# aimi-lab/robust-pose-estimator

Measured on AMD Instinct MI355X. Metric: stereo-pair pose solves/sec (640x512, 8 solver iters), higher is better.
Workload: dtype f32 (RAFT / geometry) + f64 (SE(3) solve), as the reference; 1 GPU; PoseNet.infer, 640x512 stereo frame pairs, 16 per GPU per step (RAFT batch 32), 12 GRU iters, lbfgs x8 SE(3) solve, weight heads on; frames_per_gpu=16, height=512, width=640, raft_iters=12, solver=lbfgs, solver_iters=8, parallelism=frames sharded x1

## Files before the change

include/rpe.h:

```cpp
#ifndef RPE_H
#define RPE_H

#include <stddef.h>
#include <stdint.h>

#ifdef __cplusplus
extern "C" {
#endif

#define RPE_OK 0
#define RPE_E_BADARG (-1)
#define RPE_E_LAUNCH (-2)
#define RPE_E_UNSUPPORTED (-3)

#define RPE_F32 0
#define RPE_F64 1
#define RPE_F16 2
#define RPE_F32X3 3

#define RPE_SOLVER_LBFGS 0
#define RPE_SOLVER_GN 1

#define RPE_STOP_OPT_AT_START 1
#define RPE_STOP_GTD 2
// ... 48 lines not shown
    int reserved;
} rpe_solve_opts;
#define RPE_SOLVE_LAUNCH_PER_EVALUATION 1
int rpe_pose_solve_ex(const float *flow, const float *pcl1, const float *pcl2, const float *w1, const float *w2,
                      const uint8_t *mask1, const uint8_t *mask2, const float *K, const float *loss_weight,
                      int n, int h, int w, int mode, int iters, const rpe_solve_opts *opts, double *T_out, float *vec7,
                      float *log6, int32_t *info, void *workspace, void *stream);

size_t rpe_pose_quality_workspace_bytes(int n, int h, int w);
int rpe_pose_quality(const float *flow, const float *pcl1, const float *pcl2, const float *w1, const float *w2,
                     const uint8_t *mask1, const uint8_t *mask2, const float *K, const float *loss_weight,
                     const double *T, int n, int h, int w, double *out, void *workspace, void *stream);

size_t rpe_pose_backward_workspace_bytes(int n, int h, int w);
int rpe_pose_backward_moments(const float *flow, const float *pcl1, const float *pcl2, const float *w1, const float *w2,
                              const uint8_t *mask1, const uint8_t *mask2, const float *K, const float *loss_weight,
                              const double *T, int n, int h, int w, double *out, void *workspace, void *stream);
int rpe_pose_backward_grads(const float *flow, const float *pcl1, const float *pcl2, const float *w1, const float *w2,
                            const uint8_t *mask1, const uint8_t *mask2, const float *K, const float *loss_weight,
                            const double *T, const double *u, int n, int h, int w, float *grad_flow, float *grad_pcl1,
                            float *grad_pcl2, float *grad_w1, float *grad_w2, void *stream);

int rpe_depth_backproject_warp(const float *stereo_flow2, const float *time_flow, const float *baseline,
                               const float *K, const float *depth1, const float *image1l, const float *image2l,
                               const float *stereo_flow1, const uint8_t *mask2, int n, int h, int w,
                               float *depth2, uint8_t *mask2_valid, float *pcl1, float *pcl2w, uint8_t *mask2w,
                               float *inp1, float *inp2, float *pcl2, void *stream);

int rpe_flow2depth(const float *stereo_flow, const float *baseline, int n, int h, int w, float *depth,
                   uint8_t *valid, void *stream);

int rpe_warp_taps(const float *flow, int n, int h, int w, int32_t *x0, int32_t *y0, int32_t *xn, int32_t *yn,
                  void *stream);

size_t rpe_depth_backproject_warp_backward_workspace_bytes(int n, int h, int w);
int rpe_depth_backproject_warp_backward(const float *stereo_flow2, const float *time_flow, const float *baseline,
                                        const float *K, const float *depth1, const float *image2l,
                                        const float *stereo_flow1, const uint8_t *mask2, int n, int h, int w,
                                        const float *grad_pcl1, const float *grad_pcl2w, const float *grad_inp1,
                                        const float *grad_inp2, float *grad_time_flow, float *grad_stereo_flow2,
                                        float *grad_stereo_flow1, float *grad_depth1, void *workspace, void *stream);
int rpe_flow2depth_backward(const float *stereo_flow, const float *baseline, const float *grad_depth, int n, int h, int w,
                            float *grad_stereo_flow, void *stream);

int rpe_upsample_convex_backward(const float *grad_up, const float *flow, const float *mask, int b, int h8, int w8, float *d_flow,
                                 float *d_mask, void *stream);
size_t rpe_conv_bwd_weight_workspace_bytes(int b, int cin, int cout, int h, int w, int kh, int kw);
int rpe_conv_bwd_weight(const float *x, long long x_batch_stride, const float *dy, long long dy_batch_stride, int b, int cin, int cout,
                        int h, int w, int kh, int kw, float scale, float *d_weight, float *d_bias, void *workspace, void *stream);
int rpe_conv3x3_to2_bwd_data(const float *dy, long long dy_batch_stride, const float *weight, const float *act,
                             long long act_batch_stride, int b, int c, int h, int w, float *dx, long long dx_batch_stride, void *stream);
int rpe_relu_backward(const float *grad, long long grad_batch_stride, const float *act, long long act_batch_stride, int b, int c, int hw,
                      float *out, long long out_batch_stride, void *stream);
int rpe_sum_groups(const float *parts, int groups, int b, int c, int hw, const float *bias, int relu, float *out, long long out_batch_stride,
                   void *stream);

int rpe_gru_gates_zr_recompute(const float *zr_pre, long long zr_batch_stride, const float *h, long long h_batch_stride, int b, int c, int hw,
                               float *z, long long z_batch_stride, float *r, long long r_batch_stride, float *rh, long long rh_batch_stride,
                               void *stream);
int rpe_gru_gates_h_recompute(const float *q_pre, long long qp_batch_stride, const float *z, long long z_batch_stride, const float *h,
                              long long h_batch_stride, int b, int c, int hw, float *q, long long q_batch_stride, float *h_new,
                              long long hn_batch_stride, void *stream);
int rpe_gru_gates_zq_backward(const float *d_h_new, long long d_batch_stride, const float *h, long long h_batch_stride, const float *z,
                              long long z_batch_stride, const float *q, long long q_batch_stride, int b, int c, int hw, float *d_z_pre,
                              long long dz_batch_stride, float *d_q_pre, long long dq_batch_stride, float *d_h, long long dh_batch_stride,
                              void *stream);
int rpe_gru_gates_r_backward(const float *d_rh, long long drh_batch_stride, const float *h, long long h_batch_stride, const float *r,
                             long long r_batch_stride, const float *d_h_in, long long dhi_batch_stride, int b, int c, int hw, float *d_r_pre,
                             long long dr_batch_stride, float *d_h_out, long long dho_batch_stride, void *stream);

size_t rpe_corr_grad_volume_floats(int b, int h8, int w8, int levels);
int rpe_corr_lookup_backward(const float *coords, const float *d_corr, int b, int h8, int w8, int levels, int radius, float *grad_volume,
                             void *stream);
size_t rpe_corr_build_backward_workspace_bytes(int b, int c, int h8, int w8, int levels);
int rpe_corr_build_backward(const float *grad_volume, const float *fmap1, const float *fmap2, int b, int c, int h8, int w8, int levels,
                            float *d_fmap1, float *d_fmap2, float *d_f2cat, void *workspace, void *stream);

size_t rpe_corr_pyramid_bytes(int b, int h8, int w8, int levels);
size_t rpe_corr_pyramid_bytes_ex(int b, int h8, int w8, int levels, int feature_dtype);
int rpe_corr_build(const float *fmap1, const float *fmap2, int b, int c, int h8, int w8, int levels,
                   void *pyramid, void *stream);
int rpe_corr_build_ex(const float *fmap1, const float *fmap2, int b, int c, int h8, int w8, int levels, int feature_dtype,
                      void *pyramid, void *stream);
int rpe_corr_lookup(const void *pyramid, const float *coords, int b, int h8, int w8, int levels, int radius,
                    float *out, void *stream);
int rpe_corr_lookup_ex(const void *pyramid, const float *coords, int b, int h8, int w8, int levels, int radius, int map_h, int map_w,
                       float *out, void *stream);
size_t rpe_corr_lookup_conv1x1_packed_floats(int cout, int cin);
int rpe_corr_lookup_conv1x1_pack(const float *weight, int cout, int cin, float *packed, void *stream);
int rpe_corr_lookup_conv1x1(const void *pyramid, const float *coords, int b, int h8, int w8, int levels, int radius, const float *packed,
                            const float *bias, int relu, float *out, long long out_batch_stride, float *out2, long long out2_batch_stride,
                            void *stream);
int rpe_corr_lookup_taps(const float *coords, int b, int h8, int w8, int levels, int32_t *x0, int32_t *y0,
                         void *stream);
int rpe_corr_lookup_rounds(const float *coords, int b, int h8, int w8, int levels, int32_t *rounds, int32_t *lines,
                           void *stream);
int rpe_corr_export_level(const void *pyramid, int b, int h8, int w8, int levels, int level, float *dense,
                          void *stream);

#define RPE_CORR_ALT_PAD 512
size_t rpe_corr_alt_bytes(int b, int c, int h8, int w8, int levels);
int rpe_corr_alt_prepare(const float *fmap1, const float *fmap2, int b, int c, int h8, int w8, int levels, void *scratch, void *stream);
int rpe_corr_alt_lookup(const void *scratch, const float *coords, int b, int c, int h8, int w8, int levels, int radius, float *out,
                        void *stream);
int rpe_corr_alt_lookup_ex(const void *scratch, const float *coords, int b, int c, int h8, int w8, int levels, int radius, int map_h, int map_w,
                           float *out, void *stream);
size_t rpe_corr_alt_bytes_ex(int b, int c, int h8, int w8, int levels, int feature_dtype);
int rpe_corr_alt_prepare_ex(const float *fmap1, const float *fmap2, int b, int c, int h8, int w8, int levels, int feature_dtype, void *scratch,
                            void *stream);
int rpe_corr_alt_lookup_dt(const void *scratch, const float *coords, int b, int c, int h8, int w8, int levels, int radius, int map_h, int map_w,
                           int feature_dtype, float *out, void *stream);

int rpe_gru_gates_zr(const float *zr_pre, const float *zr_bias, const float *zr_add, const float *h, int h_channels,
                     int b, int c, int hw, float *z_out, float *rh_out, int rh_channels, void *stream);
int rpe_gru_gates_h(const float *z, const float *q_pre, const float *q_bias, const float *q_add, const float *h,
                    int h_channels, int b, int c, int hw, float *h_out, int hout_channels, void *stream);
int rpe_bias_act(const float *x, const float *bias, int b, int c, int hw, int relu, float *out1, int out1_channels,
                 int out1_offset, float *out2, int out2_channels, int out2_offset, void *stream);
int rpe_instnorm_act(const float *x, const float *bias, int b, int c, int hw, float eps, int relu,
                     const float *residual, float *out, void *stream);
int rpe_affine_act(const float *x, const float *scale, const float *shift, int b, int c, int hw, int relu,
                   const float *residual, float *out, void *stream);
int rpe_copy_planes(const float *src, long long src_batch_stride, float *dst, long long dst_batch_stride, int b, int c, int hw,
                    void *stream);
int rpe_conv3x3_to2(const float *x, const float *weight, const float *bias, int b, int c, int h, int w,
                    const float *add, float *out, void *stream);
int rpe_conv3x3_to2_flow(const float *x, const float *weight, const float *bias, int b, int c, int h, int w,
                         const float *coords, float *coords_out, float *flow_out, float *dst1, long long dst1_batch_stride,
                         float *dst2, long long dst2_batch_stride, void *stream);
int rpe_flow_forward_interpolate(const float *flow, int b, int h, int w, float *out, void *stream);
int rpe_flow_seed(const float *flow_init, int b, int h, int w, float *coords_out, float *flow_out, float *dst1, long long dst1_batch_stride,
                  float *dst2, long long dst2_batch_stride, void *stream);
int rpe_upsample_convex(const float *flow, const float *mask, int b, int h8, int w8, float *out, void *stream);
int rpe_upsample_convex_ex(const float *flow, const float *mask, int b, int h8, int w8, int map_h, int map_w, float *out, void *stream);
int rpe_conv3x3_to2_flow_v(const float *x, const float *weight, const float *bias, int b, int c, int h, int w,
                           const float *coords, float *coords_out, float *flow_out, float *dst1, long long dst1_batch_stride,
                           float *dst2, long long dst2_batch_stride, int h_valid, int w_valid, void *stream);
int rpe_copy_rect(const float *src, long long src_batch_stride, long long src_plane_stride, int src_pitch, float *dst,
                  long long dst_batch_stride, long long dst_plane_stride, int dst_pitch, int b, int c, int h, int w, void *stream);

#define RPE_CONV_LINEAR 0
#define RPE_CONV_RELU 1
#define RPE_CONV_GATE_ZR 2
#define RPE_CONV_GATE_H 3
#define RPE_CONV_TANH 4
typedef struct rpe_conv_desc {
    const float *x;      long long x_batch_stride;
    const float *packed;
    const float *bias;
    const float *add;    long long add_batch_stride;
    float *out;          long long out_batch_stride;
    float *out2;         long long out2_batch_stride;
    const float *hidden; long long hidden_batch_stride;
    const float *zgate;  long long zgate_batch_stride;
    const float *scale;
    const float *residual; long long residual_batch_stride;
    float *stats;
    const float *pre_norm;
    int b, cin, cout, h, w, kh, kw, mode, gate_channels;
    int stride;
    int stats_tiles;
} rpe_conv_desc;
typedef struct rpe_conv_desc_v { rpe_conv_desc d; int h_valid, w_valid; } rpe_conv_desc_v;
int rpe_conv_wino_v(const rpe_conv_desc_v *desc, void *stream);
int rpe_conv_wino24_v(const rpe_conv_desc_v *desc, void *stream);
int rpe_conv_wino1d_v(const rpe_conv_desc_v *desc, void *stream);
int rpe_conv1x1_v(const rpe_conv_desc_v *desc, void *stream);
int rpe_enc_conv_wino_v(const rpe_conv_desc_v *desc, void *stream);
int rpe_enc_conv_wino24_v(const rpe_conv_desc_v *desc, void *stream);
int rpe_enc_conv_s2_v(const rpe_conv_desc_v *desc, void *stream);
int rpe_enc_conv_s2_m96_v(const rpe_conv_desc_v *desc, void *stream);
size_t rpe_conv_packed_floats(int cout, int cin, int kh, int kw);
int rpe_conv_pack(const float *weight, int cout, int cin, int kh, int kw, float *packed, void *stream);
int rpe_conv_fused(const rpe_conv_desc *desc, void *stream);
int rpe_conv_fused_m96(const rpe_conv_desc *desc, void *stream);
size_t rpe_conv_wino_packed_floats(int cout, int cin);
int rpe_conv_wino_stats_tiles(int h, int w);
int rpe_conv_wino_pack(const float *weight, int cout, int cin, float *packed, void *stream);
int rpe_conv_wino(const rpe_conv_desc *desc, void *stream);
size_t rpe_conv_wino24_packed_floats(int cout, int cin);
int rpe_conv_wino24_pack(const float *weight, int cout, int cin, float *packed, void *stream);
int rpe_conv_wino24(const rpe_conv_desc *desc, void *stream);
size_t rpe_conv_wino_x3_packed_bytes(int cout, int cin);
int rpe_conv_wino_x3_pack(const float *weight, int cout, int cin, void *packed, void *stream);
int rpe_conv_wino_x3(const rpe_conv_desc *desc, void *stream);
size_t rpe_conv_wino1d_packed_floats(int cout, int cin);
int rpe_conv_wino1d_pack(const float *weight, int cout, int cin, float *packed, void *stream);
int rpe_conv_wino1d(const rpe_conv_desc *desc, void *stream);
size_t rpe_conv_wino1d_x3_packed_bytes(int cout, int cin);
int rpe_conv_wino1d_x3_pack(const float *weight, int cout, int cin, void *packed, void *stream);
int rpe_conv_wino1d_x3(const rpe_conv_desc *desc, void *stream);
size_t rpe_conv1x1_packed_floats(int cout, int cin);
int rpe_conv1x1_pack(const float *weight, int cout, int cin, float *packed, void *stream);
int rpe_conv1x1(const rpe_conv_desc *desc, void *stream);
size_t rpe_conv1x1_x3_packed_bytes(int cout, int cin);
int rpe_conv1x1_x3_pack(const float *weight, int cout, int cin, void *packed, void *stream);
int rpe_conv1x1_x3(const rpe_conv_desc *desc, void *stream);
size_t rpe_conv_f16_packed_bytes(int cout, int cin, int kh, int kw);
int rpe_conv_f16_pack(const float *weight, int cout, int cin, int kh, int kw, void *packed, void *stream);
int rpe_conv_f16(const rpe_conv_desc *desc, void *stream);
int rpe_conv_direct(const float *x, long long x_batch_stride, const float *weight, const float *bias, int b, int cin, int cout,
                    int h, int w, int kh, int kw, int stride, int pad_h, int pad_w, int relu, float *out,
                    long long out_batch_stride, void *stream);
int rpe_conv_stats_tiles(int cout, int h, int w, int stride);
int rpe_conv_stats_tiles_batch(int cout, int h, int w, int stride, int b);
int rpe_instnorm_apply(const float *x, const float *partials, int tiles, int b, int c, int hw, float eps, int relu,
                       const float *residual, float *out, void *stream);
int rpe_instnorm_apply_ex(const float *x, const float *partials, int tiles, int b, int c, int hw, float eps, int relu,
                          const float *residual, const float *residual_mean_inv, float *out, void *stream);
int rpe_instnorm_finalize(const float *partials, int tiles, int b, int c, int hw, float eps, float *mean_inv, void *stream);
int rpe_instnorm_apply_v(const float *x, const float *mean_inv, int b, int c, int h, int w, int h_valid, int w_valid, int relu,
                         const float *residual, const float *residual_mean_inv, float *out, void *stream);

#define RPE_OP_CONV_FUSED 1
#define RPE_OP_CONV_WINO 2
#define RPE_OP_CONV_WINO1D 3
#define RPE_OP_CONV1X1 4
#define RPE_OP_CONV_WINO_X3 5
#define RPE_OP_CONV_WINO1D_X3 6
#define RPE_OP_CONV1X1_X3 7
#define RPE_OP_CORR_LOOKUP 8
#define RPE_OP_STEM_CONV 9
#define RPE_OP_FLOW_UPDATE 10
#define RPE_OP_COPY_PLANES 11
#define RPE_OP_INSTNORM_FINALIZE 12
#define RPE_OP_INSTNORM_APPLY 13
#define RPE_OP_UPSAMPLE_CONVEX 14
#define RPE_OP_CORR_BUILD 15
#define RPE_OP_LOOKUP_CONV1X1 16
#define RPE_OP_CONV_WINO24 17
#define RPE_OP_FLOW_SEED 18
#define RPE_OP_CONV_FUSED_M96 19
#define RPE_OP_CORR_ALT_PREPARE 20
#define RPE_OP_CORR_ALT_LOOKUP 21
#define RPE_OP_CONV_WINO_V 22
#define RPE_OP_CONV_WINO24_V 23
#define RPE_OP_CONV_WINO1D_V 24
#define RPE_OP_CONV1X1_V 25
#define RPE_OP_STEM_CONV_V 26
#define RPE_OP_FLOW_UPDATE_V 27
#define RPE_OP_CORR_LOOKUP_EX 28
#define RPE_OP_CORR_ALT_LOOKUP_EX 29
#define RPE_OP_UPSAMPLE_CONVEX_EX 30
#define RPE_OP_COPY_RECT 31
#define RPE_OP_EVENT_RECORD 32
#define RPE_OP_STREAM_WAIT 33
#define RPE_OP_ENC_CONV_WINO_V 34
#define RPE_OP_ENC_CONV_WINO24_V 35
#define RPE_OP_ENC_CONV_S2_V 36
#define RPE_OP_ENC_CONV_S2_M96_V 37
#define RPE_OP_INSTNORM_APPLY_V 38
#define RPE_OP_CORR_ALT_PREPARE_EX 39
#define RPE_OP_CORR_ALT_LOOKUP_DT 40
#define RPE_OP_CONV_F16 (RPE_OP_CORR_ALT_LOOKUP_DT + 1)
typedef struct rpe_op {
    int kind;
    int stream;
    const void *args;
} rpe_op;
typedef struct rpe_corr_lookup_args { const void *pyramid; const float *coords; int b, h8, w8, levels, radius; float *out; } rpe_corr_lookup_args;
typedef struct rpe_lookup_conv1x1_args {
    const void *pyramid; const float *coords; int b, h8, w8, levels, radius; const float *packed, *bias; int relu; float *out;
    long long out_batch_stride; float *out2; long long out2_batch_stride;
} rpe_lookup_conv1x1_args;
typedef struct rpe_corr_build_args { const float *fmap1, *fmap2; int b, c, h8, w8, levels, feature_dtype; void *pyramid; } rpe_corr_build_args;
typedef struct rpe_corr_alt_prepare_args { const float *fmap1, *fmap2; int b, c, h8, w8, levels; void *scratch; } rpe_corr_alt_prepare_args;
typedef struct rpe_corr_alt_lookup_args { const void *scratch; const float *coords; int b, c, h8, w8, levels, radius; float *out; } rpe_corr_alt_lookup_args;
typedef struct rpe_stem_conv_args {
    const float *image; int b, cin, h, w, stride; float div, mul, sub; const float *packed; int cout; const float *bias, *scale; int relu;
    float *out, *stats;
} rpe_stem_conv_args;
typedef struct rpe_flow_update_args {
    const float *x, *weight, *bias; int b, c, h, w; const float *coords; float *coords_out, *flow_out, *dst1; long long dst1_batch_stride;
    float *dst2; long long dst2_batch_stride;
} rpe_flow_update_args;
typedef struct rpe_flow_seed_args {
    const float *flow_init; int b, h, w; float *coords_out, *flow_out, *dst1; long long dst1_batch_stride; float *dst2; long long dst2_batch_stride;
} rpe_flow_seed_args;
typedef struct rpe_copy_planes_args { const float *src; long long src_batch_stride; float *dst; long long dst_batch_stride; int b, c, hw; } rpe_copy_planes_args;
typedef struct rpe_instnorm_finalize_args { const float *partials; int tiles, b, c, hw; float eps; float *mean_inv; } rpe_instnorm_finalize_args;
typedef struct rpe_instnorm_apply_args {
    const float *x, *partials; int tiles, b, c, hw; float eps; int relu; const float *residual, *residual_mean_inv; float *out;
} rpe_instnorm_apply_args;
typedef struct rpe_upsample_convex_args { const float *flow, *mask; int b, h8, w8; float *out; } rpe_upsample_convex_args;
typedef struct rpe_corr_lookup_ex_args { const void *pyramid; const float *coords; int b, h8, w8, levels, radius, map_h, map_w; float *out; } rpe_corr_lookup_ex_args;
typedef struct rpe_corr_alt_lookup_ex_args {
    const void *scratch; const float *coords; int b, c, h8, w8, levels, radius, map_h, map_w; float *out;
} rpe_corr_alt_lookup_ex_args;
typedef struct rpe_stem_conv_v_args {
    const float *image; int b, cin, h, w, stride; float div, mul, sub; const float *packed; int cout; const float *bias, *scale; int relu;
    float *out, *stats; int h_valid, w_valid;
} rpe_stem_conv_v_args;
typedef struct rpe_flow_update_v_args {
    const float *x, *weight, *bias; int b, c, h, w; const float *coords; float *coords_out, *flow_out, *dst1; long long dst1_batch_stride;
    float *dst2; long long dst2_batch_stride; int h_valid, w_valid;
} rpe_flow_update_v_args;
typedef struct rpe_upsample_convex_ex_args { const float *flow, *mask; int b, h8, w8, map_h, map_w; float *out; } rpe_upsample_convex_ex_args;
typedef struct rpe_copy_rect_args {
    const float *src; long long src_batch_stride, src_plane_stride; int src_pitch; float *dst; long long dst_batch_stride, dst_plane_stride;
    int dst_pitch, b, c, h, w;
} rpe_copy_rect_args;
typedef struct rpe_instnorm_apply_v_args {
    const float *x, *mean_inv; int b, c, h, w, h_valid, w_valid, relu; const float *residual, *residual_mean_inv; float *out;
} rpe_instnorm_apply_v_args;
typedef struct rpe_corr_alt_prepare_ex_args {
    const float *fmap1, *fmap2; int b, c, h8, w8, levels, feature_dtype; void *scratch;
} rpe_corr_alt_prepare_ex_args;
typedef struct rpe_corr_alt_lookup_dt_args {
    const void *scratch; const float *coords; int b, c, h8, w8, levels, radius, map_h, map_w, feature_dtype; float *out;
} rpe_corr_alt_lookup_dt_args;
int rpe_run_ops(const rpe_op *ops, int n_ops, void *const *streams, int n_streams, int *failed_op);

size_t rpe_unet_params_floats(int in_channels);
size_t rpe_unet_workspace_bytes(int b, int h8, int w8);
int rpe_unet_heads(const float *inp1, const float *inp2, const float *hidden, const float *context, long long hidden_batch_stride,
                   long long context_batch_stride, const float *params2d, const float *params3d, int b, int h8, int w8, int H, int W,
                   float *out2d, float *out3d, void *workspace, void *stream);

size_t rpe_unet_train_workspace_bytes(int n, int cin, int h8, int w8, int out_h, int out_w);
size_t rpe_unet_train_workspace_offset(int n, int cin, int h8, int w8, int index);
int rpe_unet_train_workspace_extent(int n, int cin, int h8, int w8, int index, int *extent);
size_t rpe_unet_train_grad_floats(int cin);
size_t rpe_unet_train_grad_offset(int cin, int index);
int rpe_unet_train_forward(const float *const *src, const int *src_channels, const long long *src_batch_strides, int nsrc,
                           const float *const *params, float *const *running_mean, float *const *running_var,
                           long long *const *num_batches_tracked, const float *momentum, const float *eps, int train_mask,
                           int n, int h8, int w8, int out_h, int out_w, int sigmoid, float *out, void *workspace, void *stream);
int rpe_unet_train_backward(const float *grad_out, const float *out, const float *const *src, const int *src_channels,
                            const long long *src_batch_strides, int nsrc, const float *const *params, int train_mask, int n, int h8, int w8,
                            int out_h, int out_w, int sigmoid, float *grad_params, float *grad_input, void *workspace, void *stream);

int rpe_stem_tiles(int h, int w, int stride);
size_t rpe_stem_packed_floats(int cout, int cin);
int rpe_stem_pack(const float *weight, int cout, int cin, float *packed, void *stream);
int rpe_stem_conv(const float *image, int b, int cin, int h, int w, int stride, float div, float mul, float sub,
                  const float *packed, int cout, const float *bias, const float *scale, int relu, float *out,
                  float *stats, void *stream);
int rpe_stem_conv_v(const float *image, int b, int cin, int h, int w, int stride, float div, float mul, float sub,
                    const float *packed, int cout, const float *bias, const float *scale, int relu, float *out,
                    float *stats, int h_valid, int w_valid, void *stream);

int rpe_mask_specularities(const uint8_t *img_hwc, const uint8_t *mask, int h, int w, int sum_threshold, uint8_t *out,
                           void *stream);
int rpe_resize_crop(const void *in, int in_is_u8_hwc, int c, int h, int w, int resized_h, int resized_w, int top, int left,
                    int out_h, int out_w, float *out, void *stream);
int rpe_resize_crop_mask(const uint8_t *in, int h, int w, int resized_h, int resized_w, int top, int left, int out_h,
                         int out_w, uint8_t *out, void *stream);
int rpe_remap_nearest(const void *src, int src_is_u8, int c, int h, int w, const float *mapx, const float *mapy, int out_h,
// ... 52 lines not shown
```

robust-pose-estimator_amd/_lib.py:

```python
import ctypes
import os
import subprocess

import torch

_HERE = os.path.dirname(os.path.abspath(__file__))
LIB_PATH = os.environ.get('RPE_HIP_LIBRARY', os.path.join(_HERE, 'librpe_hip.so'))
CSRC = os.path.join(_HERE, 'csrc')

_c = ctypes
_vp, _i, _i64, _d, _sz = _c.c_void_p, _c.c_int, _c.c_int64, _c.c_double, _c.c_size_t

_f, _ll = _c.c_void_p, _c.c_longlong


class ConvDesc(_c.Structure):
    _fields_ = [('x', _f), ('x_batch_stride', _ll), ('packed', _f), ('bias', _f), ('add', _f), ('add_batch_stride', _ll),
                ('out', _f), ('out_batch_stride', _ll), ('out2', _f), ('out2_batch_stride', _ll),
                ('hidden', _f), ('hidden_batch_stride', _ll), ('zgate', _f), ('zgate_batch_stride', _ll),
                ('scale', _f), ('residual', _f), ('residual_batch_stride', _ll), ('stats', _f), ('pre_norm', _f),
                ('b', _i), ('cin', _i), ('cout', _i), ('h', _i), ('w', _i), ('kh', _i), ('kw', _i), ('mode', _i),
                ('gate_channels', _i), ('stride', _i), ('stats_tiles', _i)]


class ConvDescV(ConvDesc):
    _fields_ = [('h_valid', _i), ('w_valid', _i)]


def struct_fields(st):
    return [f for cls in reversed(type(st).__mro__) for f in cls.__dict__.get('_fields_', ())]


class Op(_c.Structure):
    _fields_ = [('kind', _i), ('stream', _i), ('args', _vp)]


_fl = _c.c_float


class CorrLookupArgs(_c.Structure):
    _fields_ = [('pyramid', _vp), ('coords', _vp), ('b', _i), ('h8', _i), ('w8', _i), ('levels', _i), ('radius', _i), ('out', _vp)]


class LookupConv1x1Args(_c.Structure):
    _fields_ = [('pyramid', _vp), ('coords', _vp), ('b', _i), ('h8', _i), ('w8', _i), ('levels', _i), ('radius', _i), ('packed', _vp), ('bias', _vp),
                ('relu', _i), ('out', _vp), ('out_batch_stride', _ll), ('out2', _vp), ('out2_batch_stride', _ll)]


class CorrBuildArgs(_c.Structure):
    _fields_ = [('fmap1', _vp), ('fmap2', _vp), ('b', _i), ('c', _i), ('h8', _i), ('w8', _i), ('levels', _i), ('feature_dtype', _i), ('pyramid', _vp)]


class CorrAltPrepareArgs(_c.Structure):
    _fields_ = [('fmap1', _vp), ('fmap2', _vp), ('b', _i), ('c', _i), ('h8', _i), ('w8', _i), ('levels', _i), ('scratch', _vp)]


class CorrAltLookupArgs(_c.Structure):
    _fields_ = [('scratch', _vp), ('coords', _vp), ('b', _i), ('c', _i), ('h8', _i), ('w8', _i), ('levels', _i), ('radius', _i), ('out', _vp)]


class StemConvArgs(_c.Structure):
    _fields_ = [('image', _vp), ('b', _i), ('cin', _i), ('h', _i), ('w', _i), ('stride', _i), ('div', _fl), ('mul', _fl), ('sub', _fl), ('packed', _vp),
                ('cout', _i), ('bias', _vp), ('scale', _vp), ('relu', _i), ('out', _vp), ('stats', _vp)]


class FlowUpdateArgs(_c.Structure):
    _fields_ = [('x', _vp), ('weight', _vp), ('bias', _vp), ('b', _i), ('c', _i), ('h', _i), ('w', _i), ('coords', _vp), ('coords_out', _vp),
                ('flow_out', _vp), ('dst1', _vp), ('dst1_batch_stride', _ll), ('dst2', _vp), ('dst2_batch_stride', _ll)]


class CopyPlanesArgs(_c.Structure):
    _fields_ = [('src', _vp), ('src_batch_stride', _ll), ('dst', _vp), ('dst_batch_stride', _ll), ('b', _i), ('c', _i), ('hw', _i)]


class InstnormFinalizeArgs(_c.Structure):
    _fields_ = [('partials', _vp), ('tiles', _i), ('b', _i), ('c', _i), ('hw', _i), ('eps', _fl), ('mean_inv', _vp)]


class InstnormApplyArgs(_c.Structure):
    _fields_ = [('x', _vp), ('partials', _vp), ('tiles', _i), ('b', _i), ('c', _i), ('hw', _i), ('eps', _fl), ('relu', _i), ('residual', _vp),
                ('residual_mean_inv', _vp), ('out', _vp)]


class UpsampleConvexArgs(_c.Structure):
    _fields_ = [('flow', _vp), ('mask', _vp), ('b', _i), ('h8', _i), ('w8', _i), ('out', _vp)]


class FlowSeedArgs(_c.Structure):
    _fields_ = [('flow_init', _vp), ('b', _i), ('h', _i), ('w', _i), ('coords_out', _vp), ('flow_out', _vp), ('dst1', _vp), ('dst1_batch_stride', _ll),
                ('dst2', _vp), ('dst2_batch_stride', _ll)]


class CorrLookupExArgs(_c.Structure):
    _fields_ = [('pyramid', _vp), ('coords', _vp), ('b', _i), ('h8', _i), ('w8', _i), ('levels', _i), ('radius', _i), ('map_h', _i), ('map_w', _i), ('out', _vp)]


class CorrAltLookupExArgs(_c.Structure):
    _fields_ = [('scratch', _vp), ('coords', _vp), ('b', _i), ('c', _i), ('h8', _i), ('w8', _i), ('levels', _i), ('radius', _i), ('map_h', _i), ('map_w', _i),
                ('out', _vp)]


class CorrAltPrepareExArgs(_c.Structure):
    _fields_ = [('fmap1', _vp), ('fmap2', _vp), ('b', _i), ('c', _i), ('h8', _i), ('w8', _i), ('levels', _i), ('feature_dtype', _i), ('scratch', _vp)]


class CorrAltLookupDtArgs(_c.Structure):
    _fields_ = [('scratch', _vp), ('coords', _vp), ('b', _i), ('c', _i), ('h8', _i), ('w8', _i), ('levels', _i), ('radius', _i), ('map_h', _i), ('map_w', _i),
                ('feature_dtype', _i), ('out', _vp)]


class StemConvVArgs(_c.Structure):
    _fields_ = StemConvArgs._fields_ + [('h_valid', _i), ('w_valid', _i)]


class FlowUpdateVArgs(_c.Structure):
    _fields_ = FlowUpdateArgs._fields_ + [('h_valid', _i), ('w_valid', _i)]


class UpsampleConvexExArgs(_c.Structure):
    _fields_ = [('flow', _vp), ('mask', _vp), ('b', _i), ('h8', _i), ('w8', _i), ('map_h', _i), ('map_w', _i), ('out', _vp)]


class CopyRectArgs(_c.Structure):
    _fields_ = [('src', _vp), ('src_batch_stride', _ll), ('src_plane_stride', _ll), ('src_pitch', _i), ('dst', _vp), ('dst_batch_stride', _ll),
                ('dst_plane_stride', _ll), ('dst_pitch', _i), ('b', _i), ('c', _i), ('h', _i), ('w', _i)]


class InstnormApplyVArgs(_c.Structure):
    _fields_ = [('x', _vp), ('mean_inv', _vp), ('b', _i), ('c', _i), ('h', _i), ('w', _i), ('h_valid', _i), ('w_valid', _i), ('relu', _i),
                ('residual', _vp), ('residual_mean_inv', _vp), ('out', _vp)]


OP_CONV_FUSED, OP_CONV_WINO, OP_CONV_WINO1D, OP_CONV1X1, OP_CONV_WINO_X3, OP_CONV_WINO1D_X3, OP_CONV1X1_X3 = 1, 2, 3, 4, 5, 6, 7
OP_CORR_LOOKUP, OP_STEM_CONV, OP_FLOW_UPDATE, OP_COPY_PLANES, OP_INSTNORM_FINALIZE, OP_INSTNORM_APPLY, OP_UPSAMPLE_CONVEX, OP_CORR_BUILD = 8, 9, 10, 11, 12, 13, 14, 15
OP_LOOKUP_CONV1X1, OP_CONV_WINO24, OP_FLOW_SEED, OP_CONV_FUSED_M96 = 16, 17, 18, 19
OP_CORR_ALT_PREPARE, OP_CORR_ALT_LOOKUP = 20, 21
OP_CONV_WINO_V, OP_CONV_WINO24_V, OP_CONV_WINO1D_V, OP_CONV1X1_V, OP_STEM_CONV_V, OP_FLOW_UPDATE_V = 22, 23, 24, 25, 26, 27
OP_CORR_LOOKUP_EX, OP_CORR_ALT_LOOKUP_EX, OP_UPSAMPLE_CONVEX_EX, OP_COPY_RECT = 28, 29, 30, 31
OP_EVENT_RECORD, OP_STREAM_WAIT = 32, 33
OP_ENC_CONV_WINO_V, OP_ENC_CONV_WINO24_V, OP_ENC_CONV_S2_V, OP_ENC_CONV_S2_M96_V, OP_INSTNORM_APPLY_V = 34, 35, 36, 37, 38
OP_CORR_ALT_PREPARE_EX, OP_CORR_ALT_LOOKUP_DT = 39, 40
OP_CONV_F16 = 41
F32, F16 = 0, 2
LIST_OPS = {OP_CONV_FUSED: ('rpe_conv_fused', ConvDesc), OP_CONV_WINO: ('rpe_conv_wino', ConvDesc), OP_CONV_WINO1D: ('rpe_conv_wino1d', ConvDesc),
            OP_CONV1X1: ('rpe_conv1x1', ConvDesc), OP_CONV_WINO_X3: ('rpe_conv_wino_x3', ConvDesc),
            OP_CONV_WINO1D_X3: ('rpe_conv_wino1d_x3', ConvDesc), OP_CONV1X1_X3: ('rpe_conv1x1_x3', ConvDesc),
            OP_CORR_LOOKUP: ('rpe_corr_lookup', CorrLookupArgs), OP_STEM_CONV: ('rpe_stem_conv', StemConvArgs),
            OP_FLOW_UPDATE: ('rpe_conv3x3_to2_flow', FlowUpdateArgs), OP_COPY_PLANES: ('rpe_copy_planes', CopyPlanesArgs),
            OP_INSTNORM_FINALIZE: ('rpe_instnorm_finalize', InstnormFinalizeArgs), OP_INSTNORM_APPLY: ('rpe_instnorm_apply_ex', InstnormApplyArgs),
            OP_UPSAMPLE_CONVEX: ('rpe_upsample_convex', UpsampleConvexArgs), OP_CORR_BUILD: ('rpe_corr_build_ex', CorrBuildArgs),
            OP_LOOKUP_CONV1X1: ('rpe_corr_lookup_conv1x1', LookupConv1x1Args), OP_CONV_WINO24: ('rpe_conv_wino24', ConvDesc),
            OP_FLOW_SEED: ('rpe_flow_seed', FlowSeedArgs), OP_CONV_FUSED_M96: ('rpe_conv_fused_m96', ConvDesc),
            OP_CORR_ALT_PREPARE: ('rpe_corr_alt_prepare', CorrAltPrepareArgs), OP_CORR_ALT_LOOKUP: ('rpe_corr_alt_lookup', CorrAltLookupArgs),
            OP_CONV_WINO_V: ('rpe_conv_wino_v', ConvDesc), OP_CONV_WINO24_V: ('rpe_conv_wino24_v', ConvDesc),
            OP_CONV_WINO1D_V: ('rpe_conv_wino1d_v', ConvDesc), OP_CONV1X1_V: ('rpe_conv1x1_v', ConvDesc),
            OP_STEM_CONV_V: ('rpe_stem_conv_v', StemConvVArgs), OP_FLOW_UPDATE_V: ('rpe_conv3x3_to2_flow_v', FlowUpdateVArgs),
            OP_CORR_LOOKUP_EX: ('rpe_corr_lookup_ex', CorrLookupExArgs), OP_CORR_ALT_LOOKUP_EX: ('rpe_corr_alt_lookup_ex', CorrAltLookupExArgs),
            OP_UPSAMPLE_CONVEX_EX: ('rpe_upsample_convex_ex', UpsampleConvexExArgs), OP_COPY_RECT: ('rpe_copy_rect', CopyRectArgs)}
LIST_OPS_ENC = {OP_ENC_CONV_WINO_V: ('rpe_enc_conv_wino_v', ConvDesc), OP_ENC_CONV_WINO24_V: ('rpe_enc_conv_wino24_v', ConvDesc),
            OP_ENC_CONV_S2_V: ('rpe_enc_conv_s2_v', ConvDesc), OP_ENC_CONV_S2_M96_V: ('rpe_enc_conv_s2_m96_v', ConvDesc),
            OP_INSTNORM_APPLY_V: ('rpe_instnorm_apply_v', InstnormApplyVArgs)}
ENC_FORM = {'rpe_conv_wino': 'rpe_enc_conv_wino_v', 'rpe_conv_wino24': 'rpe_enc_conv_wino24_v', 'rpe_conv_fused': 'rpe_enc_conv_s2_v',
            'rpe_conv_fused_m96': 'rpe_enc_conv_s2_m96_v'}
LIST_OPS_ALT_DT = {OP_CORR_ALT_PREPARE_EX: ('rpe_corr_alt_prepare_ex', CorrAltPrepareExArgs), OP_CORR_ALT_LOOKUP_DT: ('rpe_corr_alt_lookup_dt', CorrAltLookupDtArgs)}
LIST_OPS_F16 = {OP_CONV_F16: ('rpe_conv_f16', ConvDesc)}
ALL_LIST_OPS = {**LIST_OPS, **LIST_OPS_ENC, **LIST_OPS_ALT_DT, **LIST_OPS_F16}
KIND_OF_ENTRY = {entry: kind for kind, (entry, _) in ALL_LIST_OPS.items()}

ABI_MINOR = 3
ABI_MINOR_MANY = 4
SURFEL_MAX_MAPS = 64
ABI_VERSION = 5


class SolveOpts(_c.Structure):
    _fields_ = [('struct_size', _i), ('history_size', _i), ('tolerance_grad', _d), ('tolerance_change', _d), ('partition_rows', _i), ('reserved', _i)]


class SurfelMapDesc(_c.Structure):
    _fields_ = [('opts', _vp), ('rgb', _vp), ('conf', _vp), ('t_created', _vp), ('cap', _i64), ('count', _vp), ('overflow', _vp)]


_SMP = _c.POINTER(SurfelMapDesc)
_P64, _P32, _PVP = _c.POINTER(_i64), _c.POINTER(_c.c_int32), _c.POINTER(_vp)

SIGNATURES = {
    'rpe_version': (_c.c_char_p, []),
    'rpe_abi_version': (_i, []),
    'rpe_abi_minor': (_i, []),
    'rpe_se3_exp': (_i, [_vp, _vp, _i64, _i, _vp]),
    'rpe_se3_log': (_i, [_vp, _vp, _i64, _i, _vp]),
    'rpe_se3_mul': (_i, [_vp, _vp, _vp, _i64, _i, _vp]),
    'rpe_se3_inv': (_i, [_vp, _vp, _i64, _i, _vp]),
    'rpe_se3_act': (_i, [_vp, _vp, _vp, _i64, _i64, _i, _vp]),
    'rpe_se3_chain': (_i, [_vp, _vp, _vp, _i64, _d, _i, _vp]),
    'rpe_pose_gate_chain': (_i, [_vp, _vp, _vp, _vp, _vp, _i64, _d, _d, _i, _vp]),
    'rpe_pose_gate_chain_rows': (_i, [_vp, _vp, _vp, _vp, _vp, _i64, _d, _d, _i, _vp]),
    'rpe_pose_workspace_bytes': (_sz, [_i, _i, _i]),
    'rpe_pose_reduce': (_i, [_vp] * 10 + [_i, _i, _i, _i, _vp, _vp, _vp]),
    'rpe_pose_solve': (_i, [_vp] * 9 + [_i, _i, _i, _i, _i, _vp, _vp, _vp, _vp, _vp, _vp]),
    'rpe_pose_solve_opts': (_i, [_vp] * 9 + [_i, _i, _i, _i, _i, _d, _d, _i, _vp, _vp, _vp, _vp, _vp, _vp]),
    'rpe_pose_solve_ex': (_i, [_vp] * 9 + [_i, _i, _i, _i, _i, _c.POINTER(SolveOpts), _vp, _vp, _vp, _vp, _vp, _vp]),
    'rpe_pose_quality_workspace_bytes': (_sz, [_i, _i, _i]),
    'rpe_pose_quality': (_i, [_vp] * 10 + [_i, _i, _i, _vp, _vp, _vp]),
    'rpe_pose_backward_workspace_bytes': (_sz, [_i, _i, _i]),
    'rpe_pose_backward_moments': (_i, [_vp] * 10 + [_i, _i, _i, _vp, _vp, _vp]),
    'rpe_pose_backward_grads': (_i, [_vp] * 11 + [_i, _i, _i] + [_vp] * 6),
    'rpe_depth_backproject_warp': (_i, [_vp] * 9 + [_i, _i, _i] + [_vp] * 9),
    'rpe_flow2depth': (_i, [_vp, _vp, _i, _i, _i, _vp, _vp, _vp]),
    'rpe_warp_taps': (_i, [_vp, _i, _i, _i, _vp, _vp, _vp, _vp, _vp]),
    'rpe_depth_backproject_warp_backward_workspace_bytes': (_sz, [_i, _i, _i]),
    'rpe_depth_backproject_warp_backward': (_i, [_vp] * 8 + [_i, _i, _i] + [_vp] * 10),
    'rpe_flow2depth_backward': (_i, [_vp, _vp, _vp, _i, _i, _i, _vp, _vp]),
    'rpe_upsample_convex_backward': (_i, [_vp, _vp, _vp, _i, _i, _i, _vp, _vp, _vp]),
    'rpe_conv_bwd_weight_workspace_bytes': (_sz, [_i] * 7),
    'rpe_conv_bwd_weight': (_i, [_vp, _ll, _vp, _ll] + [_i] * 7 + [_fl, _vp, _vp, _vp, _vp]),
    'rpe_conv3x3_to2_bwd_data': (_i, [_vp, _ll, _vp, _vp, _ll, _i, _i, _i, _i, _vp, _ll, _vp]),
    'rpe_relu_backward': (_i, [_vp, _ll, _vp, _ll, _i, _i, _i, _vp, _ll, _vp]),
    'rpe_sum_groups': (_i, [_vp, _i, _i, _i, _i, _vp, _i, _vp, _ll, _vp]),
    'rpe_gru_gates_zr_recompute': (_i, [_vp, _ll] * 2 + [_i, _i, _i] + [_vp, _ll] * 3 + [_vp]),
    'rpe_gru_gates_h_recompute': (_i, [_vp, _ll] * 3 + [_i, _i, _i] + [_vp, _ll] * 2 + [_vp]),
    'rpe_gru_gates_zq_backward': (_i, [_vp, _ll] * 4 + [_i, _i, _i] + [_vp, _ll] * 3 + [_vp]),
    'rpe_gru_gates_r_backward': (_i, [_vp, _ll] * 4 + [_i, _i, _i] + [_vp, _ll] * 2 + [_vp]),
    'rpe_corr_grad_volume_floats': (_sz, [_i, _i, _i, _i]),
    'rpe_corr_lookup_backward': (_i, [_vp, _vp, _i, _i, _i, _i, _i, _vp, _vp]),
    'rpe_corr_build_backward_workspace_bytes': (_sz, [_i] * 5),
    'rpe_corr_build_backward': (_i, [_vp, _vp, _vp] + [_i] * 5 + [_vp] * 5),
    'rpe_flow_forward_interpolate': (_i, [_vp, _i, _i, _i, _vp, _vp]),
    'rpe_corr_pyramid_bytes': (_sz, [_i, _i, _i, _i]),
    'rpe_corr_pyramid_bytes_ex': (_sz, [_i, _i, _i, _i, _i]),
    'rpe_corr_alt_bytes': (_sz, [_i, _i, _i, _i, _i]),
    'rpe_corr_alt_bytes_ex': (_sz, [_i, _i, _i, _i, _i, _i]),
    'rpe_corr_build': (_i, [_vp, _vp, _i, _i, _i, _i, _i, _vp, _vp]),
    'rpe_corr_lookup_conv1x1_packed_floats': (_sz, [_i, _i]),
    'rpe_corr_lookup_conv1x1_pack': (_i, [_vp, _i, _i, _vp, _vp]),
    'rpe_corr_lookup_taps': (_i, [_vp, _i, _i, _i, _i, _vp, _vp, _vp]),
    'rpe_corr_lookup_rounds': (_i, [_vp, _i, _i, _i, _i, _vp, _vp, _vp]),
    'rpe_corr_export_level': (_i, [_vp, _i, _i, _i, _i, _i, _vp, _vp]),
    'rpe_gru_gates_zr': (_i, [_vp, _vp, _vp, _vp, _i, _i, _i, _i, _vp, _vp, _i, _vp]),
    'rpe_gru_gates_h': (_i, [_vp, _vp, _vp, _vp, _vp, _i, _i, _i, _i, _vp, _i, _vp]),
    'rpe_bias_act': (_i, [_vp, _vp, _i, _i, _i, _i, _vp, _i, _i, _vp, _i, _i, _vp]),
    'rpe_instnorm_act': (_i, [_vp, _vp, _i, _i, _i, _c.c_float, _i, _vp, _vp, _vp]),
    'rpe_affine_act': (_i, [_vp, _vp, _vp, _i, _i, _i, _i, _vp, _vp, _vp]),
    'rpe_conv3x3_to2': (_i, [_vp, _vp, _vp, _i, _i, _i, _i, _vp, _vp, _vp]),
    'rpe_conv_packed_floats': (_sz, [_i, _i, _i, _i]),
    'rpe_conv_pack': (_i, [_vp, _i, _i, _i, _i, _vp, _vp]),
    'rpe_conv1x1_packed_floats': (_sz, [_i, _i]),
    'rpe_conv1x1_pack': (_i, [_vp, _i, _i, _vp, _vp]),
    'rpe_conv_direct': (_i, [_vp, _ll, _vp, _vp, _i, _i, _i, _i, _i, _i, _i, _i, _i, _i, _i, _vp, _ll, _vp]),
# ... 181 lines not shown
```

robust-pose-estimator_amd/csrc/conv1x1.hip:

```cpp
#include "wino_common.h"
#include <type_traits>

#define G1_M 128
#define G1_N 128
#define G1_K 16
#define G1_TILE (G1_K * 128)
#define G1_BIAS 4096u

typedef float f32x16 __attribute__((ext_vector_type(16)));

struct G1P {
    const float* x; long long xbs;
    const float* wp; int cin, cout, coP, hw;
    const float* bias;
    float* out; long long obs; float* out2; long long o2bs;
    int mode;
    int W, Hv, Wv;
};

__device__ __forceinline__ void dma16_2v(const float* base, unsigned v0, unsigned v1, unsigned lds_addr) {
    unsigned keep;
    base = wave_uniform(base);
    asm volatile("s_mov_b32 %0, m0\n\ts_mov_b32 m0, %4\n\ts_nop 0\n\t"
                 "global_load_lds_dwordx4 %1, %3\n\tglobal_load_lds_dwordx4 %2, %3 offset:1024\n\ts_mov_b32 m0, %0"
                 : "=&s"(keep) : "v"(v0), "v"(v1), "s"(base), "s"(lds_addr) : "memory");
}

#ifndef G1_OCC
#define G1_OCC 3
#endif
__device__ __forceinline__ void store_sv(float* base, unsigned voff, float v) {
    asm volatile("global_store_dword %0, %1, %2" :: "v"(voff), "v"(v), "s"(base) : "memory");
}

__host__ __device__ __forceinline__ int g1_chan(int rho) { return (rho >> 1) + 8 * (rho & 1); }

template <int MODE, bool OUT2, bool VALID = false>
__global__ __launch_bounds__(256, G1_OCC) void k_conv1x1(G1P P) {
    __shared__ __attribute__((aligned(16))) float As[3][G1_TILE];
    __shared__ __attribute__((aligned(16))) float Bs[3][G1_TILE];
    const int tid = threadIdx.x, lane = tid & 63, wv = __builtin_amdgcn_readfirstlane(tid >> 6);
    const int wm = wv >> 1, wn = wv & 1;
#ifndef G1_NO_XCD
    const unsigned lid = (gridDim.x & 7) == 0 ? (blockIdx.x & 7) * (gridDim.x >> 3) + (blockIdx.x >> 3) : blockIdx.x;
#else
    const unsigned lid = blockIdx.x;
#endif
    const int ncot = P.coP / G1_M;
    const int cot = lid % ncot;
    const int px0 = (lid / ncot) * G1_N, co0 = cot * G1_M, bz = blockIdx.z;
    const int hw = P.hw, cin = P.cin;
    const int nsteps = (cin + G1_K - 1) / G1_K;
    const float* xb = P.x + (size_t)bz * P.xbs;

    const float* wsrc = P.wp + ((size_t)cot * nsteps) * G1_TILE + (size_t)(4 * wv) * 128;
    const unsigned aoff = lane * 16u;
    const int bl = lane & 31, bh = lane >> 5;
    int pxl = px0 + 4 * bl; pxl = pxl + 4 <= hw ? pxl : hw - 4;
    unsigned boff[2], boff_last[2];
    bool past[2];
#pragma unroll
    for (int j = 0; j < 2; ++j) {
        const int k = g1_chan(4 * wv + 2 * j + bh);
        boff[j] = (unsigned)((size_t)k * hw + pxl) * 4u + G1_BIAS - 1024u * j;
        int kl = (nsteps - 1) * G1_K + k;
        past[j] = kl >= cin;
        kl = kl < cin ? kl : cin - 1;
        boff_last[j] = (unsigned)((size_t)(kl - (nsteps - 1) * G1_K) * hw + pxl) * 4u + G1_BIAS - 1024u * j;
    }
    const bool ragged = (cin % G1_K) != 0;
    const unsigned a_lds = lds_addr_of(&As[0][0]) + (unsigned)(4 * wv) * 512u, b_lds = lds_addr_of(&Bs[0][0]) + (unsigned)(4 * wv) * 512u;
    const float* xsrc = xb - G1_BIAS / 4;
    const size_t bstep = (size_t)G1_K * hw;
    auto issue = [&](int s, int buf) {
        const int sc = s < nsteps ? s : nsteps - 1;
        dma16x2(wsrc + (size_t)sc * G1_TILE, aoff, a_lds + (unsigned)buf * (G1_TILE * 4u));
        if (sc == nsteps - 1) dma16_2v(xsrc + (size_t)sc * bstep, boff_last[0], boff_last[1], b_lds + (unsigned)buf * (G1_TILE * 4u));
        else dma16_2v(xsrc + (size_t)sc * bstep, boff[0], boff[1], b_lds + (unsigned)buf * (G1_TILE * 4u));
    };

    f32x16 acc[2][2];
#pragma unroll
    for (int i = 0; i < 2; ++i)
#pragma unroll
        for (int j = 0; j < 2; ++j)
#pragma unroll
            for (int r = 0; r < 16; ++r) acc[i][j][r] = 0.0f;

    __shared__ float bias_s[G1_M];
    const int l31 = lane & 31, lh = lane >> 5;
    if (tid < G1_M) {
        const int co = co0 + tid;
        bias_s[tid] = (P.bias && co < P.cout) ? P.bias[co] : 0.0f;
    }

    issue(0, 0);
    issue(1, 1);
    const float* a_l = &As[0][0] + wm * 64 + l31 + lh * 128;
    const float* b_l = &Bs[0][0] + wn * 64 + l31 + lh * 128;
    auto step = [&](auto bufc, int s) {
        constexpr int BUF = decltype(bufc)::value, NB = (BUF + 2) % 3;
#ifndef G1_NO_DMA
        __builtin_amdgcn_s_waitcnt(0x0F74);
#endif
        if (ragged && s == nsteps - 1) {
#pragma unroll
            for (int j = 0; j < 2; ++j)
                if (past[j]) *(f32x4*)&Bs[BUF][(4 * wv + 2 * j) * 128 + lane * 4] = (f32x4){0.0f, 0.0f, 0.0f, 0.0f};
            __builtin_amdgcn_s_waitcnt(0xC07F);
        }
#ifndef G1_NO_BARRIER
        __builtin_amdgcn_s_barrier();
#endif
#ifndef G1_NO_DMA
        issue(s + 2, NB);
#endif
        const float* a = a_l + BUF * G1_TILE;
        const float* b = b_l + BUF * G1_TILE;
#pragma unroll
        for (int kk = 0; kk < G1_K; kk += 2) {
            const float a0 = a[kk * 128], a1 = a[kk * 128 + 32], b0 = b[kk * 128], b1 = b[kk * 128 + 32];
            acc[0][0] = __builtin_amdgcn_mfma_f32_32x32x2f32(a0, b0, acc[0][0], 0, 0, 0);
            acc[0][1] = __builtin_amdgcn_mfma_f32_32x32x2f32(a0, b1, acc[0][1], 0, 0, 0);
            acc[1][0] = __builtin_amdgcn_mfma_f32_32x32x2f32(a1, b0, acc[1][0], 0, 0, 0);
            acc[1][1] = __builtin_amdgcn_mfma_f32_32x32x2f32(a1, b1, acc[1][1], 0, 0, 0);
        }
    };
    {
        typedef std::integral_constant<int, 0> I0; typedef std::integral_constant<int, 1> I1; typedef std::integral_constant<int, 2> I2;
        int s = 0;
        while (true) {
            step(I0{}, s); if (++s == nsteps) break;
            step(I1{}, s); if (++s == nsteps) break;
            step(I2{}, s); if (++s == nsteps) break;
        }
    }
    __builtin_amdgcn_s_waitcnt(0x0F70);

    float* ob = P.out + (size_t)bz * P.obs;
    float* ob2 = OUT2 ? P.out2 + (size_t)bz * P.o2bs : nullptr;
    const int co_w = co0 + wm * 64;
    const int cout = P.cout;
    const float* bsl = &bias_s[wm * 64 + 4 * lh];
#pragma unroll
    for (int j = 0; j < 2; ++j) {
        const int px = px0 + wn * 64 + j * 32 + l31;
        const bool pok = px < hw;
        const bool pvalid = !VALID || (px / P.W < P.Hv && px % P.W < P.Wv);
        const unsigned loff = ((unsigned)(4 * lh) * (unsigned)hw + (unsigned)px) * 4u;
#pragma unroll
        for (int i = 0; i < 2; ++i)
#pragma unroll
            for (int r = 0; r < 16; ++r) {
                const int row_u = co_w + i * 32 + (r & 3) + 8 * (r >> 2);
                float v = acc[i][j][r] + bsl[i * 32 + (r & 3) + 8 * (r >> 2)];
                if (MODE == RPE_CONV_RELU) v = v < 0.0f ? 0.0f : v;
                else if (MODE == RPE_CONV_TANH) v = tanh_f(v);
                if (VALID) v = pvalid ? v : 0.0f;
#ifdef G1_NO_STORE
                if (pok && row_u + 4 * lh < cout && v == 1234.5f) {
#else
                if (pok && row_u + 4 * lh < cout) {
#endif
                    store_sv(ob + (size_t)row_u * hw, loff, v);
                    if (OUT2) store_sv(ob2 + (size_t)row_u * hw, loff, v);
                }
            }
    }
}

__global__ void k_conv1x1_pack(const float* __restrict__ w, float* __restrict__ wp, int cout, int cin, int nsteps, long long total) {
    const long long e = (long long)blockIdx.x * blockDim.x + threadIdx.x;
    if (e >= total) return;
    const int col = (int)(e & 127), k = (int)((e >> 7) & 15);
    const long long rest = e >> 11;
    const int step = (int)(rest % nsteps), tile = (int)(rest / nsteps);
    const int co = tile * 128 + col, ci = step * G1_K + g1_chan(k);
    wp[e] = (co < cout && ci < cin) ? w[(size_t)co * cin + ci] : 0.0f;
}

extern "C" size_t rpe_conv1x1_packed_floats(int cout, int cin) {
    if (cout <= 0 || cin <= 0) return 0;
    return (size_t)(round_up(cout, 128) / 128) * ceil_div(cin, G1_K) * G1_TILE;
}

extern "C" int rpe_conv1x1_pack(const float* weight, int cout, int cin, float* packed, void* stream) {
    return launch_pack(k_conv1x1_pack, weight, packed, cout, cin, 1, (long long)rpe_conv1x1_packed_floats(cout, cin), stream, ceil_div(cin, G1_K));
}

static int conv1x1_launch(const rpe_conv_desc* d, int hv, int wv, void* stream) {
    if (!conv_desc_present(d)) return RPE_E_BADARG;
    if (d->kh != 1 || d->kw != 1 || !stride_is_1(d)) return RPE_E_UNSUPPORTED;
    if (!conv_linear_or_relu(d) && d->mode != RPE_CONV_TANH) return RPE_E_UNSUPPORTED;
    if (!conv_plain_only(d) || !conv_no_encoder_epilogue(d)) return RPE_E_UNSUPPORTED;
    const long long hw = (long long)d->h * d->w;
    if ((hw & 3) || hw < 4 || !aligned16(d->x, d->x_batch_stride) || !aligned16(d->packed, 0)) return RPE_E_UNSUPPORTED;
    if (hw * 16 * 4 + G1_BIAS >= (1ll << 32)) return RPE_E_UNSUPPORTED;
    G1P P;
    fill_common(P, d, round_up(d->cout, 128));
    P.hw = (int)hw; P.W = d->w; P.Hv = hv; P.Wv = wv;
    const bool valid = hv != d->h || wv != d->w;
    const dim3 grid(ceil_div(hw, G1_N) * (P.coP / 128), 1, d->b);
#define G1_LAUNCH(M_) do { if (valid && d->out2) hipLaunchKernelGGL((k_conv1x1<M_, true, true>), grid, dim3(256), 0, (hipStream_t)stream, P); \
                           else if (valid) hipLaunchKernelGGL((k_conv1x1<M_, false, true>), grid, dim3(256), 0, (hipStream_t)stream, P); \
                           else if (d->out2) hipLaunchKernelGGL((k_conv1x1<M_, true>), grid, dim3(256), 0, (hipStream_t)stream, P); \
                           else hipLaunchKernelGGL((k_conv1x1<M_, false>), grid, dim3(256), 0, (hipStream_t)stream, P); } while (0)
    if (d->mode == RPE_CONV_RELU) G1_LAUNCH(RPE_CONV_RELU);
    else if (d->mode == RPE_CONV_TANH) G1_LAUNCH(RPE_CONV_TANH);
    else G1_LAUNCH(RPE_CONV_LINEAR);
#undef G1_LAUNCH
    return rpe_check_launch();
}

extern "C" int rpe_conv1x1(const rpe_conv_desc* d, void* stream) { return conv1x1_launch(d, d ? d->h : 0, d ? d->w : 0, stream); }

extern "C" int rpe_conv1x1_v(const rpe_conv_desc_v* dv, void* stream) {
    if (!dv || !conv_valid_extent_ok(dv)) return RPE_E_BADARG;
    return conv1x1_launch(&dv->d, dv->h_valid, dv->w_valid, stream);
}
```

robust-pose-estimator_amd/csrc/corr.hip:

```cpp
#include "rpe_common.h"
#include "sampling.h"
#include "corr_taps.h"
#include <type_traits>

#define MAX_LEVELS 4
#define GQ 8

struct PyrGeom {
    int b, h8, w8, levels;
    int gx, ngroups;
    int mp;
    int nbands, npx, np;
    int h[MAX_LEVELS], w[MAX_LEVELS], sk[MAX_LEVELS], wp[MAX_LEVELS];
    long long base[MAX_LEVELS];
    long long total;
};

static bool make_geom(int b, int h8, int w8, int levels, PyrGeom& G) {
    if (b <= 0 || h8 <= 0 || w8 <= 0 || levels <= 0 || levels > MAX_LEVELS) return false;
    G.b = b; G.h8 = h8; G.w8 = w8; G.levels = levels;
    G.gx = (w8 + GQ - 1) / GQ; G.ngroups = G.gx * h8; G.mp = (G.ngroups * GQ + 127) / 128 * 128;
    G.nbands = (h8 + 7) / 8; G.npx = (w8 + 15) / 16; G.np = G.nbands * G.npx * 128;
    long long off = 0;
    int h = h8, w = w8;
// ... 950 lines not shown
}

__global__ void k_lookup_conv_pack(const float* __restrict__ w, float* __restrict__ wp) {
    const int e = blockIdx.x * blockDim.x + threadIdx.x;
    if (e >= 4 * FZ_STEPS * 64 * 16) return;
    const int v = e & 15, lane = (e >> 4) & 63, step = (e >> 10) % FZ_STEPS, wave = (e >> 10) / FZ_STEPS;
    const int j = v >> 1, i = v & 1, l31 = lane & 31, lh = lane >> 5;
    const int co = 64 * wave + 32 * i + l31, ci = 16 * step + j + 8 * lh;
    wp[e] = ci < FZ_CIN ? w[(size_t)co * FZ_CIN + ci] : 0.0f;
}

__global__ void k_corr_taps(const float* __restrict__ coords, int32_t* x0, int32_t* y0, PyrGeom G) {
    const int l = blockIdx.y, bz = blockIdx.z;
    const int nq = G.h8 * G.w8;
    const int q = blockIdx.x * blockDim.x + threadIdx.x;
    if (q >= nq) return;
    const float inv = 1.0f / (float)(1 << l);
    const float cx = coords[((size_t)bz * 2 + 0) * nq + q] * inv;
    const float cy = coords[((size_t)bz * 2 + 1) * nq + q] * inv;
    TapAxis X, Y;
    make_taps(cx, G.w[l], X);
    make_taps(cy, G.h[l], Y);
    for (int i = 0; i < WIN; ++i) {
        size_t o = (((size_t)bz * G.levels + l) * WIN + i) * nq + q;
        x0[o] = ((X.bad >> i) & 1u) ? -1000000 : X.lo + i + (int)((X.dev >> i) & 1u);
        y0[o] = ((Y.bad >> i) & 1u) ? -1000000 : Y.lo + i + (int)((Y.dev >> i) & 1u);
    }
}

__global__ void k_corr_rounds(const float* __restrict__ coords, int32_t* __restrict__ rounds, int32_t* __restrict__ lines, PyrGeom G) {
    const int l = blockIdx.y, bz = blockIdx.z;
    const int nq = G.h8 * G.w8;
    const int lane = threadIdx.x & 63, wv = threadIdx.x >> 6;
    const int wave_g0 = (blockIdx.x * (blockDim.x >> 6) + wv) * 8;
    if (wave_g0 >= G.ngroups) return;
    const int grp = lane >> 3, k = lane & 7;
    const int Gi = wave_g0 + grp;
    const int qy = Gi / G.gx, qx = (Gi % G.gx) * GQ + k;
    const bool qok = Gi < G.ngroups && qx < G.w8;
    const int q = qok ? qy * G.w8 + qx : 0;
    const int hl = G.h[l], wl = G.w[l], wp = G.wp[l], sk = G.sk[l];
    const float inv = 1.0f / (float)(1 << l);
    TapAxis X, Y;
    make_taps(coords[((size_t)bz * 2 + 0) * nq + q] * inv, wl, X);
    make_taps(coords[((size_t)bz * 2 + 1) * nq + q] * inv, hl, Y);
    const int needw = WIN + 1 + (X.dev ? 1 : 0), needh = WIN + 1 + (Y.dev ? 1 : 0);
    const bool empty = !qok || X.lo + WIN + 1 < 0 || X.lo >= wl || Y.lo + WIN + 1 < 0 || Y.lo >= hl;
    const int sx = X.lo + sk - (k >> l);
    bool pending = !empty;
    int nr = 0, nl = 0;
    for (;;) {
        const LkRound R = plan_round(pending, Y.lo, sx, needw, needh);
        int r_lo = -R.gy0 > 0 ? -R.gy0 : 0, r_hi = hl - R.gy0 < R.nrows ? hl - R.gy0 : R.nrows;
        int x_lo = -R.gx0 > 0 ? -R.gx0 : 0, x_hi = wp - R.gx0 < R.nslots ? wp - R.gx0 : R.nslots;
        r_lo = r_lo > 16 ? 16 : r_lo; x_lo = x_lo > 16 ? 16 : x_lo;
        r_hi = r_hi < r_lo ? r_lo : r_hi; x_hi = x_hi < x_lo ? x_lo : x_hi;
        r_hi = r_hi > 12 ? 12 : r_hi;
        const int s0 = R.gx0 + x_lo, s1 = R.gx0 + x_hi;
        const int lines_row = x_hi > x_lo ? ((s1 + 3) >> 2) - (s0 >> 2) : 0;
        if (group_max(R.fits ? 1 : 0)) { nr += 1; nl += lines_row * (r_hi - r_lo); }
        pending = pending && !R.fits;
        if (!__any(pending)) break;
    }
    if (k == 0 && Gi < G.ngroups) {
        const size_t o = ((size_t)bz * G.levels + l) * G.ngroups + Gi;
        rounds[o] = nr; lines[o] = nl;
    }
}

__global__ void k_corr_export(const float* __restrict__ pyr, float* __restrict__ dense, PyrGeom G, int l) {
    const int nq = G.h8 * G.w8;
    const long long qb = blockIdx.x;
    const int bz = (int)(qb / nq), q = (int)(qb % nq);
    const int qy = q / G.w8, qx = q % G.w8;
    const int Gi = qy * G.gx + (qx >> 3), k = qx & 7;
    const int h = G.h[l], w = G.w[l], wp = G.wp[l];
    const float* g = pyr + G.base[l] + ((size_t)bz * G.ngroups + Gi) * h * ((size_t)wp * GQ) + (size_t)(G.sk[l] - (k >> l)) * GQ + k;
    for (int p = threadIdx.x; p < h * w; p += blockDim.x) {
        int y = p / w, x = p - y * w;
        dense[qb * h * w + p] = g[(size_t)y * wp * GQ + (size_t)x * GQ];
    }
}

extern "C" int rpe_corr_build_ex(const float* fmap1, const float* fmap2, int b, int c, int h8, int w8, int levels, int feature_dtype,
                                 void* pyramid, void* stream) {
    PyrGeom G;
    if (feature_dtype != RPE_F32 && feature_dtype != RPE_F16 && feature_dtype != RPE_F32X3) return RPE_E_BADARG;
    if (!fmap1 || !fmap2 || !pyramid || c <= 0 || c > 256 || c % BK != 0 || !make_geom(b, h8, w8, levels, G)) return RPE_E_BADARG;
    if (((uintptr_t)pyramid) & 15) return RPE_E_BADARG;
    hipStream_t s = (hipStream_t)stream;
    float* pyr = (float*)pyramid;
    float* Ap = pyr + G.total;
    float* Bp = Ap + (size_t)b * c * G.mp;
    if (feature_dtype == RPE_F16) {
        half4* Ah = (half4*)Ap;
        half4* Bh = Ah + (size_t)b * (c / 4) * G.mp;
        hipLaunchKernelGGL(k_permute_fmap_h, dim3(ceil_div(G.mp, 256), b * (c / 4)), dim3(256), 0, s, fmap1, Ah, c, h8, w8, 0, G.gx, G.npx, G.mp);
        hipLaunchKernelGGL(k_permute_fmap_h, dim3(ceil_div(G.np, 256), b * (c / 4)), dim3(256), 0, s, fmap2, Bh, c, h8, w8, 1, G.gx, G.npx, G.np);
        hipLaunchKernelGGL(k_corr_build_h, dim3(G.nbands, G.mp / BM, b), dim3(256), 0, s, (const half4*)Ah, (const half4*)Bh, pyr, c,
                           1.0f / sqrtf((float)c), G);
        return rpe_check_launch();
    }
    if (feature_dtype == RPE_F32X3) {
        unsigned short* A3 = (unsigned short*)Ap;
        unsigned short* B3 = A3 + (size_t)b * c * G.mp * 3;
        hipLaunchKernelGGL(k_permute_fmap_x3, dim3(ceil_div(G.mp, 256), b * (c / 8)), dim3(256), 0, s, fmap1, A3, c, h8, w8, 0, G.gx, G.npx, G.mp);
        hipLaunchKernelGGL(k_permute_fmap_x3, dim3(ceil_div(G.np, 256), b * (c / 8)), dim3(256), 0, s, fmap2, B3, c, h8, w8, 1, G.gx, G.npx, G.np);
        hipLaunchKernelGGL(k_corr_build_x3, dim3(G.nbands, G.mp / BM, b), dim3(256), 0, s, (const unsigned short*)A3, (const unsigned short*)B3, pyr, c,
                           1.0f / sqrtf((float)c), G);
        return rpe_check_launch();
    }
    const bool a_in_place = (w8 % 8 == 0) && G.mp == h8 * w8 && (((uintptr_t)fmap1) & 15) == 0;
    if (!a_in_place) hipLaunchKernelGGL(k_permute_fmap, dim3(ceil_div(G.mp, 256), b * c), dim3(256), 0, s, fmap1, Ap, h8, w8, 0, G.gx, G.npx, G.mp);
    hipLaunchKernelGGL(k_permute_fmap, dim3(ceil_div(G.np, 256), b * c), dim3(256), 0, s, fmap2, Bp, h8, w8, 1, G.gx, G.npx, G.np);
#ifndef CB_SMALL_WG
#define CB_SMALL_WG 4096
#endif
    if (!CB_CARRY || (long long)G.nbands * (G.mp / BM) * b < CB_SMALL_WG) {
        hipLaunchKernelGGL(k_corr_build<false>, dim3(G.nbands * G.npx, G.mp / BM, b), dim3(256), 0, s, a_in_place ? fmap1 : (const float*)Ap, (const float*)Bp, pyr, c,
                           1.0f / sqrtf((float)c), G);
        return rpe_check_launch();
    }
    hipLaunchKernelGGL(k_corr_build<true>, dim3(G.nbands, G.mp / BM, b), dim3(256), 0, s, a_in_place ? fmap1 : (const float*)Ap, (const float*)Bp, pyr, c,
                       1.0f / sqrtf((float)c), G);
    return rpe_check_launch();
}

extern "C" int rpe_corr_build(const float* fmap1, const float* fmap2, int b, int c, int h8, int w8, int levels,
                              void* pyramid, void* stream) {
    return rpe_corr_build_ex(fmap1, fmap2, b, c, h8, w8, levels, RPE_F32, pyramid, stream);
}

extern "C" int rpe_corr_lookup(const void* pyramid, const float* coords, int b, int h8, int w8, int levels, int radius,
                               float* out, void* stream) {
    PyrGeom G;
    if (!pyramid || !coords || !out || radius != RADIUS || !make_geom(b, h8, w8, levels, G)) return RPE_E_BADARG;
    hipLaunchKernelGGL(k_corr_lookup, dim3(ceil_div(G.ngroups, 8 * LK_WAVES), levels, b), dim3(64 * LK_WAVES), 0, (hipStream_t)stream,
                       (const float*)pyramid, coords, out, G);
    return rpe_check_launch();
}

extern "C" int rpe_corr_lookup_ex(const void* pyramid, const float* coords, int b, int h8, int w8, int levels, int radius, int map_h, int map_w,
                                  float* out, void* stream) {
    PyrGeom G;
    if (!pyramid || !coords || !out || radius != RADIUS || map_h < h8 || map_w < w8 || !make_geom(b, h8, w8, levels, G)) return RPE_E_BADARG;
    if ((long long)map_h * map_w * levels * WIN * WIN * 4 >= (1ll << 32)) return RPE_E_UNSUPPORTED;
    hipLaunchKernelGGL(k_corr_lookup_ex, dim3(ceil_div(G.ngroups, 8 * LK_WAVES), levels, b), dim3(64 * LK_WAVES), 0, (hipStream_t)stream,
                       (const float*)pyramid, coords, out, G, map_h, map_w);
    return rpe_check_launch();
}

extern "C" size_t rpe_corr_lookup_conv1x1_packed_floats(int cout, int cin) {
    return (cout == FZ_COUT && cin == FZ_CIN) ? (size_t)4 * FZ_STEPS * 64 * 16 : 0;
}

extern "C" int rpe_corr_lookup_conv1x1_pack(const float* weight, int cout, int cin, float* packed, void* stream) {
    if (!weight || !packed) return RPE_E_BADARG;
    if (cout != FZ_COUT || cin != FZ_CIN) return RPE_E_UNSUPPORTED;
    hipLaunchKernelGGL(k_lookup_conv_pack, dim3(ceil_div(4 * FZ_STEPS * 64 * 16, 256)), dim3(256), 0, (hipStream_t)stream, weight, packed);
    return rpe_check_launch();
}

extern "C" int rpe_corr_lookup_conv1x1(const void* pyramid, const float* coords, int b, int h8, int w8, int levels, int radius, const float* packed,
                                       const float* bias, int relu, float* out, long long out_batch_stride, float* out2, long long out2_batch_stride,
                                       void* stream) {
    PyrGeom G;
    if (!pyramid || !coords || !packed || !out || radius != RADIUS || !make_geom(b, h8, w8, levels, G)) return RPE_E_BADARG;
    if (levels != MAX_LEVELS || (w8 % GQ) != 0 || b > 65535) return RPE_E_UNSUPPORTED;
    FzP P{(const float*)pyramid, coords, packed, bias, out, out_batch_stride, out2, out2_batch_stride, relu};
    const int tiles_per_item = ceil_div(G.ngroups, 8);
    const long long total = (long long)tiles_per_item * b;
    int dev = 0, cus = 0;
    if (hipGetDevice(&dev) != hipSuccess || hipDeviceGetAttribute(&cus, hipDeviceAttributeMultiprocessorCount, dev) != hipSuccess || cus <= 0) cus = 256;
    if (total > cus && total < (1ll << 31)) {
        if (out2) hipLaunchKernelGGL(k_lookup_conv1x1_pipe<true>, dim3(cus), dim3(512), 0, (hipStream_t)stream, P, G, tiles_per_item, (int)total);
        else hipLaunchKernelGGL(k_lookup_conv1x1_pipe<false>, dim3(cus), dim3(512), 0, (hipStream_t)stream, P, G, tiles_per_item, (int)total);
        return rpe_check_launch();
    }
    const dim3 grid(tiles_per_item, b);
    if (out2) hipLaunchKernelGGL(k_lookup_conv1x1<true>, grid, dim3(256), 0, (hipStream_t)stream, P, G);
    else hipLaunchKernelGGL(k_lookup_conv1x1<false>, grid, dim3(256), 0, (hipStream_t)stream, P, G);
    return rpe_check_launch();
}

extern "C" int rpe_corr_lookup_taps(const float* coords, int b, int h8, int w8, int levels, int32_t* x0, int32_t* y0,
                                    void* stream) {
    PyrGeom G;
    if (!coords || !x0 || !y0 || !make_geom(b, h8, w8, levels, G)) return RPE_E_BADARG;
    const int nq = h8 * w8;
    hipLaunchKernelGGL(k_corr_taps, dim3(ceil_div(nq, 256), levels, b), dim3(256), 0, (hipStream_t)stream, coords, x0, y0, G);
    return rpe_check_launch();
}

extern "C" int rpe_corr_lookup_rounds(const float* coords, int b, int h8, int w8, int levels, int32_t* rounds, int32_t* lines,
                                      void* stream) {
    PyrGeom G;
    if (!coords || !rounds || !lines || !make_geom(b, h8, w8, levels, G)) return RPE_E_BADARG;
    hipLaunchKernelGGL(k_corr_rounds, dim3(ceil_div(G.ngroups, 8 * LK_WAVES), levels, b), dim3(64 * LK_WAVES), 0, (hipStream_t)stream,
                       coords, rounds, lines, G);
    return rpe_check_launch();
}

extern "C" int rpe_corr_export_level(const void* pyramid, int b, int h8, int w8, int levels, int level, float* dense,
                                     void* stream) {
    PyrGeom G;
    if (!pyramid || !dense || level < 0 || level >= levels || !make_geom(b, h8, w8, levels, G)) return RPE_E_BADARG;
    hipLaunchKernelGGL(k_corr_export, dim3(b * h8 * w8), dim3(256), 0, (hipStream_t)stream, (const float*)pyramid, dense, G, level);
    return rpe_check_launch();
// ... 2 lines not shown
```

robust-pose-estimator_amd/csrc/oplist.hip:

```cpp
#include "rpe_common.h"

static_assert(sizeof(rpe_op) == 16, "rpe_op: layout changed -- update _lib.py and RPE_ABI_VERSION");
static_assert(sizeof(rpe_conv_desc) == 200, "rpe_conv_desc: layout changed -- update _lib.py and RPE_ABI_VERSION");
static_assert(sizeof(rpe_corr_lookup_args) == 48, "rpe_corr_lookup_args: layout changed -- update _lib.py and RPE_ABI_VERSION");
static_assert(sizeof(rpe_corr_build_args) == 48, "rpe_corr_build_args: layout changed -- update _lib.py and RPE_ABI_VERSION");
static_assert(sizeof(rpe_corr_alt_prepare_args) == 48, "rpe_corr_alt_prepare_args: layout changed -- update _lib.py and RPE_ABI_VERSION");
static_assert(sizeof(rpe_corr_alt_lookup_args) == 48, "rpe_corr_alt_lookup_args: layout changed -- update _lib.py and RPE_ABI_VERSION");
static_assert(sizeof(rpe_stem_conv_args) == 96, "rpe_stem_conv_args: layout changed -- update _lib.py and RPE_ABI_VERSION");
static_assert(sizeof(rpe_flow_update_args) == 96, "rpe_flow_update_args: layout changed -- update _lib.py and RPE_ABI_VERSION");
static_assert(sizeof(rpe_copy_planes_args) == 48, "rpe_copy_planes_args: layout changed -- update _lib.py and RPE_ABI_VERSION");
static_assert(sizeof(rpe_instnorm_finalize_args) == 40, "rpe_instnorm_finalize_args: layout changed -- update _lib.py and RPE_ABI_VERSION");
static_assert(sizeof(rpe_instnorm_apply_args) == 64, "rpe_instnorm_apply_args: layout changed -- update _lib.py and RPE_ABI_VERSION");
static_assert(sizeof(rpe_upsample_convex_args) == 40, "rpe_upsample_convex_args: layout changed -- update _lib.py and RPE_ABI_VERSION");
static_assert(sizeof(rpe_lookup_conv1x1_args) == 96, "rpe_lookup_conv1x1_args: layout changed -- update _lib.py and RPE_ABI_VERSION");
static_assert(sizeof(rpe_flow_seed_args) == 72, "rpe_flow_seed_args: layout changed -- update _lib.py and RPE_ABI_VERSION");
static_assert(sizeof(rpe_conv_desc_v) == 208, "rpe_conv_desc_v: layout changed -- update _lib.py and RPE_ABI_VERSION");
static_assert(sizeof(rpe_corr_lookup_ex_args) == 56, "rpe_corr_lookup_ex_args: layout changed -- update _lib.py and RPE_ABI_VERSION");
static_assert(sizeof(rpe_corr_alt_lookup_ex_args) == 56, "rpe_corr_alt_lookup_ex_args: layout changed -- update _lib.py and RPE_ABI_VERSION");
static_assert(sizeof(rpe_stem_conv_v_args) == 104, "rpe_stem_conv_v_args: layout changed -- update _lib.py and RPE_ABI_VERSION");
static_assert(sizeof(rpe_flow_update_v_args) == 104, "rpe_flow_update_v_args: layout changed -- update _lib.py and RPE_ABI_VERSION");
static_assert(sizeof(rpe_upsample_convex_ex_args) == 48, "rpe_upsample_convex_ex_args: layout changed -- update _lib.py and RPE_ABI_VERSION");
static_assert(sizeof(rpe_copy_rect_args) == 80, "rpe_copy_rect_args: layout changed -- update _lib.py and RPE_ABI_VERSION");
static_assert(sizeof(rpe_instnorm_apply_v_args) == 72, "rpe_instnorm_apply_v_args: layout changed -- update _lib.py and RPE_ABI_VERSION");
static_assert(sizeof(rpe_corr_alt_prepare_ex_args) == 48, "rpe_corr_alt_prepare_ex_args: layout changed -- update _lib.py and RPE_ABI_VERSION");
static_assert(sizeof(rpe_corr_alt_lookup_dt_args) == 64, "rpe_corr_alt_lookup_dt_args: layout changed -- update _lib.py and RPE_ABI_VERSION");
static_assert(sizeof(rpe_solve_opts) == 32, "rpe_solve_opts: layout changed -- update _lib.py and RPE_ABI_VERSION");

template <typename A>
static inline const A* as(const rpe_op& op) { return static_cast<const A*>(op.args); }

static int run_one(const rpe_op& op, void* const* streams, int n_streams) {
    if (op.stream < 0 || op.stream >= n_streams || !op.args) return RPE_E_BADARG;
    void* st = streams[op.stream];
    switch (op.kind) {
    case RPE_OP_CONV_FUSED: return rpe_conv_fused(as<rpe_conv_desc>(op), st);
    case RPE_OP_CONV_FUSED_M96: return rpe_conv_fused_m96(as<rpe_conv_desc>(op), st);
    case RPE_OP_CONV_WINO: return rpe_conv_wino(as<rpe_conv_desc>(op), st);
    case RPE_OP_CONV_WINO24: return rpe_conv_wino24(as<rpe_conv_desc>(op), st);
    case RPE_OP_CONV_WINO1D: return rpe_conv_wino1d(as<rpe_conv_desc>(op), st);
    case RPE_OP_CONV1X1: return rpe_conv1x1(as<rpe_conv_desc>(op), st);
    case RPE_OP_CONV_WINO_X3: return rpe_conv_wino_x3(as<rpe_conv_desc>(op), st);
    case RPE_OP_CONV_WINO1D_X3: return rpe_conv_wino1d_x3(as<rpe_conv_desc>(op), st);
    case RPE_OP_CONV1X1_X3: return rpe_conv1x1_x3(as<rpe_conv_desc>(op), st);
    case RPE_OP_CONV_F16: return rpe_conv_f16(as<rpe_conv_desc>(op), st);
    case RPE_OP_CORR_LOOKUP: {
        const auto* a = as<rpe_corr_lookup_args>(op);
        return rpe_corr_lookup(a->pyramid, a->coords, a->b, a->h8, a->w8, a->levels, a->radius, a->out, st);
    }
    case RPE_OP_LOOKUP_CONV1X1: {
        const auto* a = as<rpe_lookup_conv1x1_args>(op);
        return rpe_corr_lookup_conv1x1(a->pyramid, a->coords, a->b, a->h8, a->w8, a->levels, a->radius, a->packed, a->bias, a->relu, a->out,
                                       a->out_batch_stride, a->out2, a->out2_batch_stride, st);
    }
    case RPE_OP_CORR_BUILD: {
        const auto* a = as<rpe_corr_build_args>(op);
        return rpe_corr_build_ex(a->fmap1, a->fmap2, a->b, a->c, a->h8, a->w8, a->levels, a->feature_dtype, a->pyramid, st);
    }
    case RPE_OP_CORR_ALT_PREPARE: {
        const auto* a = as<rpe_corr_alt_prepare_args>(op);
        return rpe_corr_alt_prepare(a->fmap1, a->fmap2, a->b, a->c, a->h8, a->w8, a->levels, a->scratch, st);
    }
    case RPE_OP_CORR_ALT_LOOKUP: {
        const auto* a = as<rpe_corr_alt_lookup_args>(op);
        return rpe_corr_alt_lookup(a->scratch, a->coords, a->b, a->c, a->h8, a->w8, a->levels, a->radius, a->out, st);
    }
    case RPE_OP_STEM_CONV: {
        const auto* a = as<rpe_stem_conv_args>(op);
        return rpe_stem_conv(a->image, a->b, a->cin, a->h, a->w, a->stride, a->div, a->mul, a->sub, a->packed, a->cout, a->bias, a->scale, a->relu,
                             a->out, a->stats, st);
    }
    case RPE_OP_FLOW_UPDATE: {
        const auto* a = as<rpe_flow_update_args>(op);
        return rpe_conv3x3_to2_flow(a->x, a->weight, a->bias, a->b, a->c, a->h, a->w, a->coords, a->coords_out, a->flow_out, a->dst1,
                                    a->dst1_batch_stride, a->dst2, a->dst2_batch_stride, st);
    }
    case RPE_OP_COPY_PLANES: {
        const auto* a = as<rpe_copy_planes_args>(op);
        return rpe_copy_planes(a->src, a->src_batch_stride, a->dst, a->dst_batch_stride, a->b, a->c, a->hw, st);
    }
    case RPE_OP_INSTNORM_FINALIZE: {
        const auto* a = as<rpe_instnorm_finalize_args>(op);
        return rpe_instnorm_finalize(a->partials, a->tiles, a->b, a->c, a->hw, a->eps, a->mean_inv, st);
    }
    case RPE_OP_INSTNORM_APPLY: {
        const auto* a = as<rpe_instnorm_apply_args>(op);
        return rpe_instnorm_apply_ex(a->x, a->partials, a->tiles, a->b, a->c, a->hw, a->eps, a->relu, a->residual, a->residual_mean_inv, a->out, st);
    }
    case RPE_OP_UPSAMPLE_CONVEX: {
        const auto* a = as<rpe_upsample_convex_args>(op);
        return rpe_upsample_convex(a->flow, a->mask, a->b, a->h8, a->w8, a->out, st);
    }
    case RPE_OP_FLOW_SEED: {
        const auto* a = as<rpe_flow_seed_args>(op);
        return rpe_flow_seed(a->flow_init, a->b, a->h, a->w, a->coords_out, a->flow_out, a->dst1, a->dst1_batch_stride, a->dst2,
                             a->dst2_batch_stride, st);
    }
    case RPE_OP_CONV_WINO_V: return rpe_conv_wino_v(as<rpe_conv_desc_v>(op), st);
    case RPE_OP_CONV_WINO24_V: return rpe_conv_wino24_v(as<rpe_conv_desc_v>(op), st);
    case RPE_OP_CONV_WINO1D_V: return rpe_conv_wino1d_v(as<rpe_conv_desc_v>(op), st);
    case RPE_OP_CONV1X1_V: return rpe_conv1x1_v(as<rpe_conv_desc_v>(op), st);
    case RPE_OP_STEM_CONV_V: {
        const auto* a = as<rpe_stem_conv_v_args>(op);
        return rpe_stem_conv_v(a->image, a->b, a->cin, a->h, a->w, a->stride, a->div, a->mul, a->sub, a->packed, a->cout, a->bias, a->scale, a->relu,
                               a->out, a->stats, a->h_valid, a->w_valid, st);
    }
    case RPE_OP_FLOW_UPDATE_V: {
        const auto* a = as<rpe_flow_update_v_args>(op);
        return rpe_conv3x3_to2_flow_v(a->x, a->weight, a->bias, a->b, a->c, a->h, a->w, a->coords, a->coords_out, a->flow_out, a->dst1,
                                      a->dst1_batch_stride, a->dst2, a->dst2_batch_stride, a->h_valid, a->w_valid, st);
    }
    case RPE_OP_CORR_LOOKUP_EX: {
        const auto* a = as<rpe_corr_lookup_ex_args>(op);
        return rpe_corr_lookup_ex(a->pyramid, a->coords, a->b, a->h8, a->w8, a->levels, a->radius, a->map_h, a->map_w, a->out, st);
    }
    case RPE_OP_CORR_ALT_LOOKUP_EX: {
        const auto* a = as<rpe_corr_alt_lookup_ex_args>(op);
        return rpe_corr_alt_lookup_ex(a->scratch, a->coords, a->b, a->c, a->h8, a->w8, a->levels, a->radius, a->map_h, a->map_w, a->out, st);
    }
    case RPE_OP_UPSAMPLE_CONVEX_EX: {
        const auto* a = as<rpe_upsample_convex_ex_args>(op);
        return rpe_upsample_convex_ex(a->flow, a->mask, a->b, a->h8, a->w8, a->map_h, a->map_w, a->out, st);
    }
    case RPE_OP_COPY_RECT: {
        const auto* a = as<rpe_copy_rect_args>(op);
        return rpe_copy_rect(a->src, a->src_batch_stride, a->src_plane_stride, a->src_pitch, a->dst, a->dst_batch_stride, a->dst_plane_stride,
                             a->dst_pitch, a->b, a->c, a->h, a->w, st);
    }
    case RPE_OP_ENC_CONV_WINO_V: return rpe_enc_conv_wino_v(as<rpe_conv_desc_v>(op), st);
    case RPE_OP_ENC_CONV_WINO24_V: return rpe_enc_conv_wino24_v(as<rpe_conv_desc_v>(op), st);
    case RPE_OP_ENC_CONV_S2_V: return rpe_enc_conv_s2_v(as<rpe_conv_desc_v>(op), st);
    case RPE_OP_ENC_CONV_S2_M96_V: return rpe_enc_conv_s2_m96_v(as<rpe_conv_desc_v>(op), st);
    case RPE_OP_INSTNORM_APPLY_V: {
        const auto* a = as<rpe_instnorm_apply_v_args>(op);
        return rpe_instnorm_apply_v(a->x, a->mean_inv, a->b, a->c, a->h, a->w, a->h_valid, a->w_valid, a->relu, a->residual, a->residual_mean_inv, a->out, st);
    }
    case RPE_OP_CORR_ALT_PREPARE_EX: {
        const auto* a = as<rpe_corr_alt_prepare_ex_args>(op);
        return rpe_corr_alt_prepare_ex(a->fmap1, a->fmap2, a->b, a->c, a->h8, a->w8, a->levels, a->feature_dtype, a->scratch, st);
    }
    case RPE_OP_CORR_ALT_LOOKUP_DT: {
        const auto* a = as<rpe_corr_alt_lookup_dt_args>(op);
        return rpe_corr_alt_lookup_dt(a->scratch, a->coords, a->b, a->c, a->h8, a->w8, a->levels, a->radius, a->map_h, a->map_w, a->feature_dtype,
                                      a->out, st);
    }
    case RPE_OP_EVENT_RECORD: {
        hipEvent_t ev = (hipEvent_t) * static_cast<void* const*>(op.args);
        if (!ev) return RPE_OK;
        return hipEventRecord(ev, (hipStream_t)st) == hipSuccess ? RPE_OK : RPE_E_LAUNCH;
    }
    case RPE_OP_STREAM_WAIT: {
        hipEvent_t ev = (hipEvent_t) * static_cast<void* const*>(op.args);
        if (!ev) return RPE_OK;
        return hipStreamWaitEvent((hipStream_t)st, ev, 0) == hipSuccess ? RPE_OK : RPE_E_LAUNCH;
    }
    default: return RPE_E_BADARG;
    }
}

extern "C" int rpe_run_ops(const rpe_op* ops, int n_ops, void* const* streams, int n_streams, int* failed_op) {
    if (failed_op) *failed_op = -1;
    if (!ops || n_ops < 0 || !streams || n_streams <= 0) return RPE_E_BADARG;
    for (int i = 0; i < n_ops; ++i) {
        const int st = run_one(ops[i], streams, n_streams);
        if (st != RPE_OK) {
            if (failed_op) *failed_op = i;
            return st;
        }
    }
    return RPE_OK;
}
```

robust-pose-estimator_amd/ops.py:

```python
import ctypes
import operator

import torch

from . import _lib
from ._lib import check, lib, ptr, stream_ptr

SOLVER_LBFGS, SOLVER_GN = 0, 1


class OpList:

    def __init__(self, n_cells=0):
        self._items, self._keep, self._arr = [], [], None
        self.cells = (ctypes.c_void_p * max(1, n_cells))()
        self._streams = (ctypes.c_void_p * 4)()
        self._failed = ctypes.c_int(-1)

    def __len__(self):
        return len(self._items)

    def add(self, launcher, stream=0):
        kind, args = launcher.op
        self._items.append((kind, stream, ctypes.addressof(args)))
        self._keep.append(launcher)
        self._arr = None
        return self

    def _cell_op(self, kind, cell, stream):
        self._items.append((kind, stream, ctypes.addressof(self.cells) + ctypes.sizeof(ctypes.c_void_p) * cell))
        self._arr = None
        return self

    def record(self, cell, stream=0):
        return self._cell_op(_lib.OP_EVENT_RECORD, cell, stream)

    def wait(self, cell, stream=0):
        return self._cell_op(_lib.OP_STREAM_WAIT, cell, stream)

    def mark(self):
        return len(self._items)

    def run(self, streams, start=0, stop=None):
        if self._arr is None:
            self._arr = (_lib.Op * max(1, len(self._items)))(*[_lib.Op(k, s, a) for k, s, a in self._items])
        stop = len(self._items) if stop is None else stop
        if stop <= start:
            return
        for i, h in enumerate(streams):
            self._streams[i] = h
        st = lib().rpe_run_ops(ctypes.cast(ctypes.byref(self._arr, ctypes.sizeof(_lib.Op) * start), ctypes.POINTER(_lib.Op)), stop - start, self._streams,
                               len(streams), ctypes.byref(self._failed))
        if st != 0:
            check(st, f'rpe_run_ops (op {start + self._failed.value} of the list, kind {self._items[start + self._failed.value][0]})')


_REC = None


class Recorder(OpList):

    def __init__(self):
        super().__init__()
        self._structs, self._bound, self._claimed = [], {}, set()
        self.complete = False

    def __enter__(self):
        global _REC
        if _REC is not None:
            raise _lib.RpeError('Recorder: recordings do not nest')
        self._count = _lib.CountingLib().__enter__()
        _REC = self
        return self

    def __exit__(self, *exc):
        global _REC
        _REC = None
        self._count.__exit__(*exc)
        self.complete = exc[0] is None and self._count.calls == len(self._items)
        self.unlogged = [] if self.complete else sorted(set(self._count.names))
        del self._count
        return False

    def log(self, kind, args, keep):
# ... 321 lines not shown
    f32 = torch.float32
    sf2 = _dev(stereo_flow2, f32, 'stereo_flow2')
    n, _, h, w = sf2.shape
    tf, b, K = _dev(time_flow, f32, 'time_flow'), _dev(baseline, f32, 'baseline'), _dev(K, f32, 'K')
    d1, i2 = _dev(depth1, f32, 'depth1'), _dev(image2l, f32, 'image2l')
    sf1, m2 = _dev(stereo_flow1, f32, 'stereo_flow1'), _mask(mask2, 'mask2')
    gin = [None if g is None else _dev(g, f32, nm) for g, nm in ((grad_pcl1, 'grad_pcl1'), (grad_pcl2w, 'grad_pcl2w'), (grad_inp1, 'grad_inp1'),
                                                                 (grad_inp2, 'grad_inp2'))]
    for g, shape in zip(gin, ((n, 3, h, w), (n, 3, h, w), (n, 8, h // 8, w // 8), (n, 8, h // 8, w // 8))):
        if g is not None and tuple(g.shape) != shape:
            raise _lib.RpeError(f'depth_backproject_warp_backward: an incoming gradient has shape {tuple(g.shape)}, expected {shape}')
    unknown = [k for k in want if k not in GEOMETRY_GRADS]
    if unknown:
        raise _lib.RpeError(f'depth_backproject_warp_backward: unknown gradients {unknown}')
    ch = dict(time_flow=2, stereo_flow2=2, stereo_flow1=2, depth1=1)
    outs = {k: (torch.empty(n, ch[k], h, w, dtype=f32, device=sf2.device) if k in want else None) for k in GEOMETRY_GRADS}
    ws = torch.empty(lib().rpe_depth_backproject_warp_backward_workspace_bytes(n, h, w), dtype=torch.uint8, device=sf2.device)
    check(lib().rpe_depth_backproject_warp_backward(ptr(sf2), ptr(tf), ptr(b), ptr(K), ptr(d1), ptr(i2), ptr(sf1), ptr(m2), n, h, w,
                                                    *[ptr(g) for g in gin], *[ptr(outs[k]) for k in GEOMETRY_GRADS], ptr(ws),
                                                    stream_ptr()), 'rpe_depth_backproject_warp_backward')
    return {k: v for k, v in outs.items() if v is not None}


def flow2depth_backward(stereo_flow, baseline, grad_depth):
    sf = _dev(stereo_flow, torch.float32, 'stereo_flow')
    n, _, h, w = sf.shape
    b, gd = _dev(baseline, torch.float32, 'baseline'), _dev(grad_depth, torch.float32, 'grad_depth')
    out = torch.empty_like(sf)
    check(lib().rpe_flow2depth_backward(ptr(sf), ptr(b), ptr(gd), n, h, w, ptr(out), stream_ptr()), 'rpe_flow2depth_backward')
    return out


class _GeometryStageFn(torch.autograd.Function):

    @staticmethod
    def forward(ctx, stereo_flow2, time_flow, baseline, K, depth1, image1l, image2l, stereo_flow1, mask2):
        g = depth_backproject_warp(stereo_flow2, time_flow, baseline, K, depth1, image1l, image2l, stereo_flow1, mask2)
        ctx.save_for_backward(stereo_flow2, time_flow, baseline, K, depth1, image2l, stereo_flow1, mask2)
        ctx.mark_non_differentiable(g['depth2'], g['mask2'], g['mask2w'])
        ctx.set_materialize_grads(False)
        return g['pcl1'], g['pcl2w'], g['inp1'], g['inp2'], g['depth2'], g['mask2'], g['mask2w']

    @staticmethod
    def backward(ctx, g_pcl1, g_pcl2w, g_inp1, g_inp2, *_):
        need = ctx.needs_input_grad
        names = {'stereo_flow2': need[0], 'time_flow': need[1], 'depth1': need[4], 'stereo_flow1': need[7]}
        want = [k for k in GEOMETRY_GRADS if names[k]]
        g = depth_backproject_warp_backward(*ctx.saved_tensors, g_pcl1, g_pcl2w, g_inp1, g_inp2, want=want) if want else {}
        return (g.get('stereo_flow2'), g.get('time_flow'), None, None, g.get('depth1'), None, None, g.get('stereo_flow1'), None)


def geometry_stage(stereo_flow2, time_flow, baseline, K, depth1, image1l, image2l, stereo_flow1, mask2):
    pcl1, pcl2w, inp1, inp2, depth2, m2v, m2w = _GeometryStageFn.apply(stereo_flow2, time_flow, baseline, K, depth1, image1l, image2l,
                                                                        stereo_flow1, mask2)
    return dict(depth2=depth2, mask2=m2v, pcl1=pcl1, pcl2w=pcl2w, mask2w=m2w, inp1=inp1, inp2=inp2, pcl2=None)


class _Flow2DepthFn(torch.autograd.Function):
    @staticmethod
    def forward(ctx, stereo_flow, baseline):
        depth, valid = flow2depth(stereo_flow, baseline)
        ctx.save_for_backward(stereo_flow, baseline)
        ctx.mark_non_differentiable(valid)
        ctx.set_materialize_grads(False)
        return depth, valid

    @staticmethod
    def backward(ctx, g_depth, _):
        return (None if g_depth is None else flow2depth_backward(*ctx.saved_tensors, g_depth)), None


def flow2depth_grad(stereo_flow, baseline):
    return _Flow2DepthFn.apply(stereo_flow, baseline)


class CorrPyramid:

    def __init__(self, b, h8, w8, levels=4, radius=4, device='cuda', bf16x3=False):
        self.b, self.h8, self.w8, self.levels, self.radius = b, h8, w8, levels, radius
        nbytes = lib().rpe_corr_pyramid_bytes_ex(b, h8, w8, levels, 3 if bf16x3 else 0)
        if nbytes == 0:
            raise _lib.RpeError('rpe_corr_pyramid_bytes: unsupported geometry')
        self.buf = torch.empty(nbytes, dtype=torch.uint8, device=device)

    def build(self, fmap1, fmap2, fp16_features=False, bf16x3=False):
        f1, f2 = _dev(fmap1, torch.float32, 'fmap1'), _dev(fmap2, torch.float32, 'fmap2')
        b, c, h8, w8 = f1.shape
        if (b, h8, w8) != (self.b, self.h8, self.w8) or f2.shape != f1.shape:
            raise _lib.RpeError('corr build: shape mismatch')
        mode = 2 if fp16_features else 3 if bf16x3 else 0
        if self.buf.numel() < lib().rpe_corr_pyramid_bytes_ex(b, h8, w8, self.levels, mode):
            raise _lib.RpeError('corr build: this pyramid was not sized for the requested feature mode (CorrPyramid(..., bf16x3=True))')
        return _launch(_lib.OP_CORR_BUILD, (ptr(f1), ptr(f2), b, c, h8, w8, self.levels, mode, ptr(self.buf)), (f1, f2, self), self)

    def lookup(self, coords, out=None, prepare=False, map_size=None):
        co = _dev(coords, torch.float32, 'coords')
        ch = self.levels * (2 * self.radius + 1) ** 2
        if map_size is not None:
            return _lookup_ex(self, _lib.OP_CORR_LOOKUP_EX, (ptr(self.buf), ptr(co), self.b, self.h8, self.w8, self.levels, self.radius), coords, co, out, ch,
                              map_size, prepare)
        if tuple(co.shape) != (self.b, 2, self.h8, self.w8):
            raise _lib.RpeError('corr lookup: coords shape mismatch')
        if out is None:
            out = torch.empty(self.b, ch, self.h8, self.w8, dtype=torch.float32, device=co.device)
        if prepare and (co is not coords or tuple(_nchw(out, 'out').shape) != (self.b, ch, self.h8, self.w8)):
            raise _lib.RpeError('corr lookup: a prepared launch needs contiguous coords and a (b, levels*(2r+1)^2, h8, w8) out buffer')
        return _launch(_lib.OP_CORR_LOOKUP, (ptr(self.buf), ptr(co), self.b, self.h8, self.w8, self.levels, self.radius, ptr(out)), (self, co, out), out,
                       prepare)

    def lookup_conv1x1(self, coords, packed, out, out2=None, relu=True, prepare=False):
        co = _dev(coords, torch.float32, 'coords')
        if co is not coords or tuple(co.shape) != (self.b, 2, self.h8, self.w8):
            raise _lib.RpeError('corr lookup_conv1x1: coords must be a contiguous (b,2,h8,w8) tensor')
        if not PackedLookupConv.supported(self.levels, self.radius, self.w8):
            raise _lib.RpeError('corr lookup_conv1x1: needs 4 levels, radius 4 and w8 % 8 == 0 (use lookup + conv1x1)')
        sl = _opt_slices('corr lookup_conv1x1', self.b, packed.cout, self.h8, self.w8, out=out, out2=out2)
        return _launch(_lib.OP_LOOKUP_CONV1X1, (ptr(self.buf), ptr(co), self.b, self.h8, self.w8, self.levels, self.radius, ptr(packed.packed),
                                                ptr(packed.bias), int(bool(relu)), *sl), (self, co, packed, out, out2), out, prepare)

    def taps(self, coords):
        co = _dev(coords, torch.float32, 'coords')
        win = 2 * self.radius + 1
        x0 = torch.empty(self.b, self.levels, win, self.h8 * self.w8, dtype=torch.int32, device=co.device)
        y0 = torch.empty_like(x0)
        check(lib().rpe_corr_lookup_taps(ptr(co), self.b, self.h8, self.w8, self.levels, ptr(x0), ptr(y0), stream_ptr()),
              'rpe_corr_lookup_taps')
        return x0, y0

    def rounds(self, coords):
        co = _dev(coords, torch.float32, 'coords')
        ng = self.h8 * ((self.w8 + 7) // 8)
        rounds = torch.zeros(self.b, self.levels, ng, dtype=torch.int32, device=co.device)
        lines = torch.zeros_like(rounds)
        check(lib().rpe_corr_lookup_rounds(ptr(co), self.b, self.h8, self.w8, self.levels, ptr(rounds), ptr(lines), stream_ptr()),
              'rpe_corr_lookup_rounds')
        return rounds, lines

    def export_level(self, level):
        h, w = self.h8 >> level, self.w8 >> level
        dense = torch.empty(self.b * self.h8 * self.w8, h, w, dtype=torch.float32, device=self.buf.device)
        check(lib().rpe_corr_export_level(ptr(self.buf), self.b, self.h8, self.w8, self.levels, level, ptr(dense),
                                          stream_ptr()), 'rpe_corr_export_level')
        return dense


class AltCorr:

    def __init__(self, b, c, h8, w8, levels=4, radius=4, device='cuda', fp16=False):
        self.b, self.c, self.h8, self.w8, self.levels, self.radius, self.fp16 = b, c, h8, w8, levels, radius, bool(fp16)
        self.nbytes = lib().rpe_corr_alt_bytes_ex(b, c, h8, w8, levels, _lib.F16 if self.fp16 else _lib.F32)
        if self.nbytes == 0 or radius != 4:
            raise _lib.RpeError('rpe_corr_alt_bytes: unsupported geometry')
        self.buf = torch.empty(self.nbytes, dtype=torch.uint8, device=device)

    def build(self, fmap1, fmap2):
        f1, f2 = _dev(fmap1, torch.float32, 'fmap1'), _dev(fmap2, torch.float32, 'fmap2')
        if tuple(f1.shape) != (self.b, self.c, self.h8, self.w8) or f2.shape != f1.shape:
            raise _lib.RpeError('corr alt build: shape mismatch')
        if self.fp16:
            return _launch(_lib.OP_CORR_ALT_PREPARE_EX, (ptr(f1), ptr(f2), self.b, self.c, self.h8, self.w8, self.levels, _lib.F16, ptr(self.buf)), (f1, f2, self),
                           self)
        return _launch(_lib.OP_CORR_ALT_PREPARE, (ptr(f1), ptr(f2), self.b, self.c, self.h8, self.w8, self.levels, ptr(self.buf)), (f1, f2, self), self)

    def lookup(self, coords, out=None, prepare=False, map_size=None):
        co = _dev(coords, torch.float32, 'coords')
        ch = self.levels * (2 * self.radius + 1) ** 2
        if map_size is not None:
            return _lookup_ex(self, _lib.OP_CORR_ALT_LOOKUP_DT if self.fp16 else _lib.OP_CORR_ALT_LOOKUP_EX,
                              (ptr(self.buf), ptr(co), self.b, self.c, self.h8, self.w8, self.levels, self.radius), coords, co, out, ch, map_size, prepare,
                              tail=(_lib.F16,) if self.fp16 else ())
        if tuple(co.shape) != (self.b, 2, self.h8, self.w8):
            raise _lib.RpeError('corr alt lookup: coords shape mismatch')
        if out is None:
            out = torch.empty(self.b, ch, self.h8, self.w8, dtype=torch.float32, device=co.device)
        if prepare and co is not coords:
# ... 203 lines not shown
    if size is not None:
        mh, mw, (h8, w8) = h8, w8, size
        if tuple(mk.shape) != (b, 576, mh, mw) or not (0 < h8 <= mh and 0 < w8 <= mw):
            raise _lib.RpeError('upsample_convex: mask must be (b,576,mh,mw) like the flow map, size within it')
        out = torch.empty(b, 2, 8 * h8, 8 * w8, dtype=torch.float32, device=fl.device)
        return _launch(_lib.OP_UPSAMPLE_CONVEX_EX, (ptr(fl), ptr(mk), b, h8, w8, mh, mw, ptr(out)), (fl, mk, out), out)
    if tuple(mk.shape) != (b, 576, h8, w8):
        raise _lib.RpeError('upsample_convex: mask must be (b,576,h/8,w/8)')
    out = torch.empty(b, 2, 8 * h8, 8 * w8, dtype=torch.float32, device=fl.device)
    return _launch(_lib.OP_UPSAMPLE_CONVEX, (ptr(fl), ptr(mk), b, h8, w8, ptr(out)), (fl, mk, out), out)


CONV_LINEAR, CONV_RELU, CONV_GATE_ZR, CONV_GATE_H, CONV_TANH = 0, 1, 2, 3, 4


def _chan_slice(t, name):
    if not (isinstance(t, torch.Tensor) and t.is_cuda and t.dtype == torch.float32 and t.dim() == 4):
        raise _lib.RpeError(f'{name}: expected a float32 NCHW tensor on the GPU')
    _, _, hh, ww = t.shape
    if t.stride(3) != 1 or t.stride(2) != ww or t.stride(1) != hh * ww:
        raise _lib.RpeError(f'{name}: expected a channel slice of a contiguous NCHW buffer')
    _on_current_device(t, name)
    return ptr(t), t.stride(0)


def _opt_slices(who, b, c, hh, ww, **named):
    sl = []
    for name, t in named.items():
        if t is None:
            sl += [None, 0]
        elif tuple(t.shape) != (b, c, hh, ww):
            raise _lib.RpeError(f'{who}: {name} must be a ({b},{c},{hh},{ww}) channel slice')
        else:
            sl += _chan_slice(t, f'{who}: {name}')
    return sl


class PackedConv(_Packed):
    error = 'needs a non-empty (cout, cin, kh, kw) weight'
    size, pack, entry = 'rpe_conv_packed_floats', 'rpe_conv_pack', 'rpe_conv_fused'

    def _dims(self):
        return self.cout, self.cin, self.kh, self.kw

    def _fits(self):
        return True

    @staticmethod
    def supported(weight, width):
        _, _, kh, kw = weight.shape
        return kh % 2 == 1 and kw in (1, 3, 5) and width % 4 == 0


class PackedConv1x1(_Packed):
    kernels, error = ((1, 1),), 'weight must be (cout, cin, 1, 1)'
    size, pack, entry = 'rpe_conv1x1_packed_floats', 'rpe_conv1x1_pack', 'rpe_conv1x1'

    @staticmethod
    def supported(h, w):
        return (h * w) % 4 == 0 and h * w >= 4


class PackedConv1x1X3(_Packed):
    kernels, error, in_bytes = ((1, 1),), 'weight must be (cout, cin, 1, 1)', True
    size, pack, entry = 'rpe_conv1x1_x3_packed_bytes', 'rpe_conv1x1_x3_pack', 'rpe_conv1x1_x3'


class PackedConvF16(_Packed):
    kernels, error, in_bytes = ((1, 1), (3, 3), (1, 5), (5, 1)), 'needs a (cout, cin, kh, kw) weight with (kh, kw) in 1x1, 3x3, 1x5, 5x1', True
    size, pack, entry = 'rpe_conv_f16_packed_bytes', 'rpe_conv_f16_pack', 'rpe_conv_f16'

    def _dims(self):
        return self.cout, self.cin, self.kh, self.kw

    @staticmethod
    def supported(weight, h, w):
        return tuple(weight.shape[2:]) in PackedConvF16.kernels and h > 0 and w > 0 and w % 4 == 0


def conv1x1(x, pc, mode, out, out2=None, prepare=False, valid=None):
    return conv_fused(x, pc, mode, out, out2=out2, prepare=prepare, entry=pc.entry, valid=valid)


class Conv1x1:

    def __init__(self, weight, bias=None):
        self._w = _nchw(weight.detach().contiguous(), 'weight')
        self._b = None if bias is None else _nchw(bias.detach().contiguous(), 'bias')
        self.cout, self.cin = self._w.shape[0], self._w.shape[1]
        self._packings = {}

    def _packing(self, cls):
        p = self._packings.get(cls)
        if p is None:
            p = self._packings[cls] = cls(self._w, self._b)
        return p

    fused = property(lambda self: self._packing(PackedConv))
    gemm = property(lambda self: self._packing(PackedConv1x1))
    gemm_x3 = property(lambda self: self._packing(PackedConv1x1X3))
    f16 = property(lambda self: self._packing(PackedConvF16))

    def __call__(self, x, mode, out, out2=None, prepare=False, x3=False, valid=None, f16=False):
        b, _, hh, ww = x.shape
        if f16:
            if x3 or valid is not None:
                raise _lib.RpeError('Conv1x1: f16 runs on rpe_conv_f16 alone -- not with x3, and there is no valid-extent form of it')
            return conv_fused(x, self.f16, mode, out, out2=out2, prepare=prepare)
        aligned = PackedConv1x1.supported(hh, ww) and x.data_ptr() % 16 == 0 and x.stride(0) % 4 == 0
        big = b * -(-(hh * ww) // 128) * -(-self.cout // 128) >= 512 and aligned
        if aligned and x3 and mode in (CONV_LINEAR, CONV_RELU):
            return conv1x1(x, self.gemm_x3, mode, out, out2=out2, prepare=prepare)
        if valid is not None:
            if not aligned or x3:
                raise _lib.RpeError('Conv1x1: a valid extent needs the f32 GEMM route (16-byte aligned input slice, h * w % 4 == 0, no bf16x3)')
            return conv1x1(x, self.gemm, mode, out, out2=out2, prepare=prepare, valid=valid)
        if big:
            return conv1x1(x, self.gemm, mode, out, out2=out2, prepare=prepare)
        return conv_fused(x, self.fused, mode, out, out2=out2, prepare=prepare)


_PLAIN_RULES = dict(add=('exact', 'cout', False), out=('min', 'cout', True), out2=('min', 'cout', False), residual=('exact', 'cout', False))
_FUSED_RULES = {CONV_GATE_ZR: dict(add=('exact', 'cout', False), out=('min', 'gate', True), out2=('min', 'gate', True), hidden=('min', 'gate', True)),
                CONV_GATE_H: dict(add=('exact', 'cout', False), out=('min', 'cout', True), hidden=('min', 'cout', True), zgate=('min', 'cout', True))}
_WINO_RULES = dict(out=('min', 'cout', True), out2=('min', 'cout', False), residual=('min', 'cout', False))
_FUSED_MODES = (CONV_LINEAR, CONV_RELU, CONV_GATE_ZR, CONV_GATE_H, CONV_TANH)


def conv_fused(x, pc, mode, out, out2=None, add=None, hidden=None, zgate=None, gate_channels=0, scale=None, bias='packed',
               residual=None, stats=None, stride=1, pre_norm=None, prepare=False, entry='rpe_conv_fused', valid=None, enc_valid=None):
    if enc_valid is not None:
        if valid is not None or stride != 2:
            raise _lib.RpeError('conv_fused: enc_valid is the stride-2 encoder form (not with valid=)')
        valid = enc_valid
    if isinstance(pc, PackedConvF16):
        entry = pc.entry
    d, bias, stats = _conv_desc('conv_fused', x, pc, mode, dict(add=add, out=out, out2=out2, hidden=hidden, zgate=zgate, residual=residual),
                                _FUSED_RULES.get(mode, _PLAIN_RULES), scale, bias, stats, pre_norm, modes=_FUSED_MODES, tile_major=False,
                                kernel=(pc.kh, pc.kw), stride=stride, gate_channels=gate_channels, valid=valid)
    return _launch(_kind(entry, valid, enc_valid is not None), d, (x, pc, out, out2, add, hidden, zgate, scale, bias, residual, stats, pre_norm), out, prepare)


def _kind(entry, valid, enc=False):
    if valid is None:
        return _lib.KIND_OF_ENTRY[entry]
    if enc:
        if entry not in _lib.ENC_FORM:
            raise _lib.RpeError(f'{entry} has no encoder valid-extent form')
        return _lib.KIND_OF_ENTRY[_lib.ENC_FORM[entry]]
    if entry + '_v' not in _lib.KIND_OF_ENTRY:
        raise _lib.RpeError(f'{entry} has no valid-extent form')
    return _lib.KIND_OF_ENTRY[entry + '_v']


def _conv_desc(who, x, pc, mode, slices, rules, scale, bias, stats, pre_norm, *, modes, tile_major, kernel, stride=1, gate_channels=0, valid=None):
    d = _lib.ConvDesc() if valid is None else _lib.ConvDescV()
    b, cin, hh, ww = x.shape
    if valid is not None:
        d.h_valid, d.w_valid = _valid_extent(who, valid, hh // stride, ww // stride)
    cout = pc.cout
    if cin != pc.cin:
        raise _lib.RpeError(f'{who}: input has {cin} channels, weights expect {pc.cin}')
    if mode not in modes:
        raise _lib.RpeError(f'{who}: mode {mode} is not an epilogue of this kernel' + (' (LINEAR / RELU only)' if len(modes) == 2 else ''))
    d.x, d.x_batch_stride = _chan_slice(x, f'{who}: x')
    bias = pc.bias if isinstance(bias, str) else bias
    for name, t in (('bias', bias), ('scale', scale)):
        if t is not None:
            _f32(t, f'{who}: {name}', numel=cout)
    d.packed, d.bias, d.scale = ptr(pc.packed), ptr(bias), ptr(scale)
    for name, t in slices.items():
        rule, kind, required = rules.get(name, ('min', None, False))
        channels = {'cout': cout, 'gate': gate_channels, None: 0}[kind]
        if t is None:
            if required:
                raise _lib.RpeError(f'{who}: this epilogue needs {name}')
            continue
        if t.shape[0] != b or tuple(t.shape[2:]) != (hh // stride, ww // stride) or (rule == 'exact' and t.shape[1] != channels):
            raise _lib.RpeError(f'{who}: {name} has shape {tuple(t.shape)}')
        if t.shape[1] < channels:
            raise _lib.RpeError(f'{who}: {name} has too few channels ({t.shape[1]}, the epilogue writes or reads {channels})')
        p, s = _chan_slice(t, f'{who}: {name}')
        setattr(d, name, p); setattr(d, name + '_batch_stride', s)
    if stats is not None:
        if isinstance(stats, TileMajorStats) != tile_major:
            raise _lib.RpeError(f'{who}: stats must come from ' + ('conv_wino_stats_buffer (tile-major records)' if tile_major else
                                                                  'conv_stats_buffer (a channel-major tensor)'))
        if tile_major:
            stats = _f32(stats.tensor, f'{who}: stats', (b, lib().rpe_conv_wino_stats_tiles(hh, ww), cout, 3))
        else:
            d.stats_tiles = lib().rpe_conv_stats_tiles(cout, hh, ww, stride)
            _f32(stats, f'{who}: stats', (b, cout, d.stats_tiles, 3))
    if pre_norm is not None:
        _f32(pre_norm, f'{who}: pre_norm', (b, cin, 2))
    d.stats, d.pre_norm = ptr(stats), ptr(pre_norm)
    d.b, d.cin, d.cout, d.h, d.w, (d.kh, d.kw), d.mode, d.gate_channels, d.stride = b, cin, cout, hh, ww, kernel, mode, gate_channels, stride
    return d, bias, stats


# ... 471 lines not shown
```

robust-pose-estimator_amd/pose_net.py:

```python
import torch
import torch.nn as nn

from . import ops, raft_grad
from .pose_head import DeclarativeLayerLie, DPoseSE3Head, create_img_coords_t
from .raft import RAFT
from .se3 import SE3
from .unet import TinyUNet, pack_params

FUSED_HEADS = True


class PoseNet(nn.Module):
    def __init__(self, config):
        super().__init__()
        self.config = config
        self.loss_weight = nn.Parameter(torch.tensor([1.0, 1.0]))
        H, W = config['image_shape']
        self.register_buffer('img_coords', create_img_coords_t(y=H, x=W), persistent=False)
        self.use_weights = config.get('use_weights', True)
        self.flow = RAFT(config)
        self.flow.freeze_bn()
        self.pose_head = DeclarativeLayerLie(DPoseSE3Head(self.img_coords, config.get('lbgfs_iters', 100),
                                                          solver=config.get('solver', 'lbfgs')))
        self.weight_head_2d = nn.Sequential(TinyUNet(in_channels=128 + 128 + 8, output_size=(H, W)), nn.Sigmoid())
# ... 20 lines not shown
            r, rec = self.flow.grad_pass((f[:n], f[n:]), cn, stages=grad, upsample=upsample)
        else:
            r = self.flow(None, None, upsample=upsample, fmaps=(f[:n], f[n:]), cnet=cn)
        flow = r[0][-1]
        depth, valid = ops.flow2depth(flow, baseline if upsample else baseline / 8.0)
        if grad is not None:
            return depth, flow, valid, rec.rows(0, n)
        if ret_cache:
            return depth, flow, valid, dict(fmap=f[:n], cnet=cn)
        return depth, flow, valid

    def forward(self, image1l, image2l, intrinsics, baseline, image1r, image2r, mask1=None, mask2=None, ret_confmap=False, ret_flows=False,
                grad_corr=False):
        n = image1l.shape[0]
        intrinsics = intrinsics.expand(n, 3, 3).contiguous()
        baseline = baseline.expand(n).contiguous()
        if grad_corr and not ret_flows:
            raise ValueError('PoseNet.forward: grad_corr returns its leaves in the dict of ret_flows: it needs ret_flows=True')
        grad = 'corr' if grad_corr else 'update' if self.flow_update_trainable() else 'heads' if self.flow_heads_trainable() else None
        if grad is not None:
            self.flow.check_grad(grad)
        with torch.no_grad():
            pass1 = None
            if grad is not None:
                depth1, stereo_flow1, valid1, pass1 = self.flow2depth(image1l, image1r, baseline, grad=grad)
            else:
                depth1, stereo_flow1, valid1 = self.flow2depth(image1l, image1r, baseline)
            mask1 = (mask1.bool() & valid1) if mask1 is not None else valid1
            mask2 = mask2.bool().clone() if mask2 is not None else torch.ones_like(valid1)
            s = self.stages(image1l, image2l, intrinsics, baseline, depth1, image2r, mask1, mask2, stereo_flow1, heads=False,
                            grad_flows=ret_flows or grad is not None, pass1=pass1)
        if self.use_weights and self.train_heads_hip:
            w2d = self.weight_head_2d[0].forward_train_hip((s['inp1'], s['hidden'], s['context']), sigmoid=True)
            w3d = self.weight_head_3d[0].forward_train_hip((s['inp1'], s['inp2'], s['hidden'], s['context']), sigmoid=True)
        elif self.use_weights:
            w2d = self.weight_head_2d(torch.cat((s['inp1'], s['hidden'], s['context']), dim=1))
            w3d = self.weight_head_3d(torch.cat((s['inp1'], s['inp2'], s['hidden'], s['context']), dim=1))
        else:
            w2d, w3d = torch.ones_like(s['depth2']), torch.ones_like(s['depth2'])
        _, log6 = self.pose_head(s['time_flow'], s['pcl1'], s['pcl2w'], w2d, w3d, mask1, s['mask2w'], s['intrinsics'],
                                 self.loss_weight.repeat(n, 1))
        pose_tan = log6.squeeze(1)
        out = (pose_tan, depth1, s['depth2'], (w2d, w3d)) if ret_confmap else (pose_tan, depth1, s['depth2'])
        if ret_flows:
            flows = {k: s[k] for k in ('time_flow', 'stereo_flow1', 'stereo_flow2')}
            flows.update({k: s[k + '_leaves'] for k in raft_grad.GradPass.LEAVES if k + '_leaves' in s})
            out = (*out, flows)
        return out

    def flow_head_params(self):
        fh, mk = self.flow.head_params()
        return fh + mk

    def flow_heads_trainable(self):
        return any(p.requires_grad for p in self.flow_head_params())

    def flow_update_trainable(self):
        params = getattr(self.flow, 'update_params', None)
        return params is not None and any(p.requires_grad for p in params())

    def freeze_flow(self, freeze=True, parts=None):
        if parts not in (None, 'heads', 'update'):
            raise ValueError(f"freeze_flow: parts must be None, 'heads' or 'update', got {parts!r}")
        if not freeze and parts == 'heads':
            for p in self.flow_head_params():
                p.requires_grad = True
            return self
        if not freeze and parts == 'update':
            for p in self.flow.update_block.parameters():
                p.requires_grad = True
            return self
        if not freeze:
            raise NotImplementedError('training the whole flow network (freeze_flow(False)) is out of scope: the gradients stop at the flows '
                                      '(forward(..., ret_flows=True) returns them), at RAFT\'s output heads (parts=\'heads\') or at its update '
                                      'block (parts=\'update\'), and through the correlation at the feature maps (grad_corr=True); the two '
                                      'encoders have no backward here')
        for p in self.parameters():
            p.requires_grad = True
        for p in self.flow.parameters():
            p.requires_grad = False
        return self

    @torch.no_grad()
    def _encode_both(self, feature_images, context_images):
        both = getattr(self.flow, 'encode_both', None)
        if both is not None:
            return both(feature_images, context_images)
        return self.flow.encode_features(feature_images), self.flow.encode_context(context_images)

    def _heads(self, g, hidden, context):
        if not self.use_weights:
            return torch.ones_like(g['depth2']), torch.ones_like(g['depth2'])
        if FUSED_HEADS and not (self.weight_head_2d.training or self.weight_head_3d.training):
            return ops.unet_heads(g['inp1'], g['inp2'], hidden, context, pack_params(self.weight_head_2d[0]),
                                  pack_params(self.weight_head_3d[0]), self.config['image_shape'])
        return (self.weight_head_2d(torch.cat((g['inp1'], hidden, context), dim=1)),
                self.weight_head_3d(torch.cat((g['inp1'], g['inp2'], hidden, context), dim=1)))

    def _solve(self, inputs, rows_alone=False):
        problem = self.pose_head.problem
        keep = problem.partition_rows
        if rows_alone:
            problem.partition_rows = 1
        try:
            return self.pose_head(*inputs)[0]
        finally:
            problem.partition_rows = keep

    @torch.no_grad()
    def stages(self, image1l, image2l, intrinsics, baseline, depth1, image2r, mask1, mask2, stereo_flow1, cache1=None, heads=True, enc2=None,
               flow_init=None, ret_lowres=False, grad_flows=False, pass1=None):
        n = image1l.shape[0]
        intrinsics = intrinsics.expand(n, 3, 3).contiguous()
        baseline = baseline.expand(n).contiguous()
        if cache1 is None:
            f, cn = self._encode_both((image1l, image2l, image2r), (image1l, image2l))
            f2l = f[n:2 * n]
            fmaps = (f[:2 * n], f[n:])
            c2l = cn[n:]
        else:
            f, c2l = (enc2['f'], enc2['c']) if enc2 is not None else self._encode_both((image2l, image2r), image2l)
            f2l = f[:n]
            fmaps = (torch.cat((cache1['fmap'], f2l), dim=0), f)
            cn = torch.cat((cache1['cnet'], c2l), dim=0)
        kw = {}
        if flow_init is not None:
            kw['flow_init'] = torch.cat((flow_init, torch.zeros_like(flow_init)), dim=0)
        if pass1 is not None:
            r, rec2 = self.flow.grad_pass(fmaps, cn, stages=pass1.depth, upsample=True, **kw)
        else:
            r = self.flow(None, None, upsample=True, fmaps=fmaps, cnet=cn, ret_lowres=ret_lowres, **kw)
        flow_predictions, hidden, context = r[:3]
        time_flow = flow_predictions[-1][:n].contiguous()
        stereo_flow2 = flow_predictions[-1][n:].contiguous()
        hidden, context = hidden[:n], context[:n]
        passes = None
        if grad_flows:
            with torch.enable_grad():
                if pass1 is not None:
                    passes = dict(time=rec2.rows(0, n), stereo1=pass1, stereo2=rec2.rows(n, 2 * n))
                    hidden = passes['time'].hidden
                    time_flow, stereo_flow1, stereo_flow2 = raft_grad.attach(
                        list(passes.values()), self.flow.head_params(), None if pass1.depth == 'heads' else self.flow.update_params())
                    for t in (time_flow, stereo_flow1, stereo_flow2):
                        t.retain_grad()
                else:
                    time_flow, stereo_flow2, stereo_flow1 = (t.detach().requires_grad_(True) for t in (time_flow, stereo_flow2, stereo_flow1))
                g = ops.geometry_stage(stereo_flow2, time_flow, baseline, intrinsics, ops.flow2depth_grad(stereo_flow1, baseline)[0],
                                       image1l, image2l, stereo_flow1, mask2)
            g['stereo_flow1'] = stereo_flow1
        else:
            g = ops.depth_backproject_warp(stereo_flow2, time_flow, baseline, intrinsics, depth1, image1l, image2l,
                                           stereo_flow1, mask2)
        w2d, w3d = self._heads(g, hidden, context) if heads else (None, None)
        g.update(time_flow=time_flow, stereo_flow2=stereo_flow2, hidden=hidden, context=context, w2d=w2d, w3d=w3d,
                 intrinsics=intrinsics, cache2=dict(fmap=f2l, cnet=c2l))
        if passes is not None:
            g.update({k + '_leaves': {p: getattr(rec, k) for p, rec in passes.items()} for k in raft_grad.GradPass.LEAVES if getattr(pass1, k) is not None})
        if ret_lowres:
            g['time_flow_low'] = g['cache2']['time_flow_low'] = r[3][:n]
        return g

    @torch.no_grad()
    def infer(self, image1l, image2l, intrinsics, baseline, depth1, image2r, mask1, mask2, stereo_flow1,
              ret_details=False, cache1=None, ret_cache=False, enc2=None, flow_init=None, ret_lowres=False, ret_quality=False, rows_alone=False):
        if enc2 is not None and cache1 is None:
            raise ValueError('infer: enc2 (the new frame encoded ahead of the call) needs cache1 (the previous frame\'s encoder outputs)')
        if ret_lowres and not ret_cache:
            raise ValueError("infer: ret_lowres returns the temporal 1/8 flow in the cache dict ('time_flow_low'): it needs ret_cache=True")
        if ret_quality and not ret_details:
            raise ValueError('infer: ret_quality adds the quality report to the details: it needs ret_details=True')
        s = self.stages(image1l, image2l, intrinsics, baseline, depth1, image2r, mask1, mask2, stereo_flow1, cache1, enc2=enc2,
                        flow_init=flow_init, ret_lowres=ret_lowres)
        mask2.copy_(s['mask2'])
        n = image1l.shape[0]
        lw = self.loss_weight.detach()[None, :].repeat(n, 1)
        inputs = (s['time_flow'], s['pcl1'], s['pcl2w'], s['w2d'], s['w3d'], mask1.bool(), s['mask2w'], s['intrinsics'], lw)
        vec7 = self._solve(inputs, rows_alone)
        pose = SE3(vec7[:, 0]) if n > 1 else SE3(vec7)[0]
        out = (pose, depth1, s['depth2'], (s['w2d'], s['w3d']), s['time_flow'], s['stereo_flow2']) if ret_details else pose
        if ret_quality:
            out = (*out, self._quality(inputs))
        if ret_cache:
            return (*out, s['cache2']) if ret_details else (out, s['cache2'])
        return out

    def _quality(self, inputs):
        problem = self.pose_head.problem
        q = ops.quality_fields(problem.quality(*inputs))
        info = problem.last_info
        d = {k: q[k] for k in ('cov', 'pd', 'n2d', 'n3d', 'rms2d_px', 'rms3d', 'f', 'grad_max')}
        d.update(n_iter=info[:, 0], func_evals=info[:, 1], stop_reason=info[:, 2])
        return d

    @torch.no_grad()
    def infer_chunk(self, image0l, imagesl, imagesr, intrinsics, baseline, depth0, mask0, masks, stereo_flow0, cache0=None,
                    depth_roundtrip=None, ret_quality=False):
        c = imagesl.shape[0]
        intrinsics = intrinsics.expand(c, 3, 3).contiguous()
# ... 39 lines not shown
```

robust-pose-estimator_amd/raft.py:

```python
import operator
from types import SimpleNamespace
from typing import NamedTuple, Optional, Tuple

import torch
import torch.nn as nn

from . import ops, raft_grad
from ._lib import RpeError
from .ops import bounded_put, wkey

WINOGRAD = True
WINO_2X4 = True
S2_M96 = True
S2_M96_MIN_WGS = 512
CORR_BF16X3 = False
CONV_BF16X3 = False
X3_MIN_CIN = 128
X3_GRU = False
UPDATE_FP16 = False
SIDE_STREAM = True
PAD_MAPS = False
PAD_ENCODERS = False
LOOP_OPLIST = True
LOOKUP_EVENT_SINK = None
FRAME_OPLISTS = True
LOOKUP_FUSED = True
LOOKUP_FUSED_MAX_WGS = 256
FRAME_OPLISTS_MAX_IMAGES = 4
ENC_STREAMS = True
ENC_STREAMS_MIN = 8
SIDE_STREAM_MAX = 8 * 5120
ROUTE_SWITCHES = ('WINOGRAD', 'WINO_2X4', 'S2_M96', 'S2_M96_MIN_WGS', 'CORR_BF16X3', 'CONV_BF16X3', 'X3_MIN_CIN', 'X3_GRU', 'SIDE_STREAM', 'SIDE_STREAM_MAX',
                  'LOOKUP_FUSED', 'LOOKUP_FUSED_MAX_WGS', 'ENC_STREAMS', 'ENC_STREAMS_MIN', 'PAD_MAPS', 'PAD_ENCODERS', 'UPDATE_FP16')
_switch_values = operator.itemgetter(*ROUTE_SWITCHES)


def _switches():
    return _switch_values(globals())


def padded_size(h8, w8):
    return h8 + (h8 & 1), (w8 + 3) // 4 * 4


class Route(NamedTuple):
    mixed_precision: bool = False
    alternate_corr: bool = False
    alt_corr_fp16: bool = False
    pad_maps: bool = False
    pad_encoders: bool = False
    update_fp16: bool = False
    loop_pad: Optional[Tuple[int, int]] = None
    enc_pad: Optional[Tuple[int, int]] = None
    fused: Optional[bool] = None

    @property
    def options(self):
        return Route(*self[:6])


def _fused(w8, update_fp16):
    if w8 % 4 != 0 and update_fp16:
        raise RpeError(f'RAFT: update_fp16 needs a 1/8 map with w % 4 == 0 (rpe_conv_f16), got w8 = {w8}; it does not run in f32 instead')
    return w8 % 4 == 0


def resolve_route(mixed_precision=False, alternate_corr=False, alt_corr_fp16=False, pad_maps=False, pad_encoders=False, update_fp16=False,
                  map_size=None, image_size=None):
    pad_maps, pad_encoders, update_fp16 = bool(pad_maps or PAD_MAPS), bool(pad_encoders or PAD_ENCODERS), bool(update_fp16 or UPDATE_FP16)
    if alt_corr_fp16 and not alternate_corr:
        raise RpeError('RAFT: alt_corr_fp16 selects the feature precision of alternate_corr and needs alternate_corr: True')
    if alternate_corr and (mixed_precision or CORR_BF16X3 or CONV_BF16X3):
        raise RpeError('RAFT: alternate_corr is f32 only (fp16 features: alt_corr_fp16) -- not with mixed_precision, CORR_BF16X3 or CONV_BF16X3')
    if pad_maps and (CONV_BF16X3 or not WINOGRAD):
        raise RpeError('RAFT: pad_maps runs on the f32 Winograd kernels -- not with CONV_BF16X3 (X3_GRU), not without WINOGRAD')
    if pad_encoders and (CONV_BF16X3 or not WINOGRAD):
        raise RpeError('RAFT: pad_encoders runs on the f32 Winograd kernels -- not with CONV_BF16X3, not without WINOGRAD')
    if update_fp16 and CONV_BF16X3:
        raise RpeError('RAFT: update_fp16 and CONV_BF16X3 are two precisions for the same layers -- choose one')
    if update_fp16 and not WINOGRAD:
        raise RpeError('RAFT: update_fp16 keeps its f32 layers on the Winograd kernels -- not with WINOGRAD = False')
    if update_fp16 and (pad_maps or pad_encoders):
        raise RpeError('RAFT: update_fp16 has no valid-extent form yet -- not with pad_maps / pad_encoders')
    options = (bool(mixed_precision), bool(alternate_corr), bool(alt_corr_fp16), pad_maps, pad_encoders, update_fp16)
    if image_size is not None:
        map_size = image_size[0] // 8, image_size[1] // 8
    if map_size is None:
        return Route(*options)
    padded = padded_size(*map_size)
    padded = None if padded == tuple(map_size) else padded
    loop_pad = padded if pad_maps else None
    enc_pad = padded if pad_encoders and image_size is not None and image_size[0] % 8 == 0 and image_size[1] % 8 == 0 else None
    return Route(*options, loop_pad, enc_pad, _fused((loop_pad or map_size)[1], update_fp16))


def _norm(kind, ch):
    if kind == 'batch':
        return nn.BatchNorm2d(ch)
    if kind == 'instance':
        return nn.InstanceNorm2d(ch)
    if kind == 'none':
        return nn.Sequential()
    raise ValueError(kind)


class ResidualBlock(nn.Module):
    def __init__(self, in_planes, planes, norm_fn='batch', stride=1):
        super().__init__()
        self.conv1 = nn.Conv2d(in_planes, planes, kernel_size=3, padding=1, stride=stride)
        self.conv2 = nn.Conv2d(planes, planes, kernel_size=3, padding=1)
        self.relu = nn.ReLU(inplace=True)
        self.norm1 = _norm(norm_fn, planes)
        self.norm2 = _norm(norm_fn, planes)
# ... 121 lines not shown


class _Recorded:

    def __init__(self, keep=4):
        self._progs, self._failed, self._keep = {}, {}, keep

    def get(self, key):
        return self._progs.get(key)

    def wanted(self, key):
        return self._failed.get(key, 0) < 3

    def put(self, key, rec):
        if rec.complete:
            bounded_put(self._progs, key, rec, keep=self._keep)
        else:
            if len(self._failed) > 64:
                self._failed.clear()
            self._failed[key] = self._failed.get(key, 0) + 1

    def clear(self):
        self._progs.clear()
        self._failed.clear()


class BasicEncoder(nn.Module):
    def __init__(self, output_dim=128, norm_fn='batch', dropout=0.0, pad_encoders=False):
        super().__init__()
        self.norm_fn = norm_fn
        self.pad_encoders = pad_encoders
        self.norm1 = _norm(norm_fn, 64)
        self.conv1 = nn.Conv2d(3, 64, kernel_size=7, stride=2, padding=3)
        self.relu1 = nn.ReLU(inplace=True)
        self.in_planes = 64
        self.layer1 = self._make_layer(64, stride=1)
        self.layer2 = self._make_layer(96, stride=2)
        self.layer3 = self._make_layer(128, stride=2)
        self.conv2 = nn.Conv2d(128, output_dim, kernel_size=1)
        for m in self.modules():
            if isinstance(m, nn.Conv2d):
                nn.init.kaiming_normal_(m.weight, mode='fan_out', nonlinearity='relu')
            elif isinstance(m, (nn.BatchNorm2d, nn.InstanceNorm2d)):
                if m.weight is not None:
                    nn.init.constant_(m.weight, 1)
                if m.bias is not None:
                    nn.init.constant_(m.bias, 0)

    def _make_layer(self, dim, stride=1):
        l1 = ResidualBlock(self.in_planes, dim, self.norm_fn, stride=stride)
        l2 = ResidualBlock(dim, dim, self.norm_fn, stride=1)
        self.in_planes = dim
        return nn.Sequential(l1, l2)

    def _stem_pack(self):
        w = self.conv1.weight
        return _cached(self, '_stem_packed', wkey(w), lambda: ops.PackedStem(w))

    def _stem_many(self, images):
        ps = self._stem_pack()
        n = sum(im.shape[0] for im in images)
        hh, ww = images[0].shape[-2:]
        out = torch.empty(n, 64, hh // 2, ww // 2, device=images[0].device)
        bn = isinstance(self.norm1, nn.BatchNorm2d)
        if bn:
            if self.norm1.training:
                raise RuntimeError('the RAFT encoders run with frozen batch norm (RAFT.freeze_bn, pose_net.py:22)')
            scale, shift = _bn_affine(self.conv1, self.norm1)
        stats = None if bn else torch.empty(n, 64, ops.lib().rpe_stem_tiles(hh, ww, 2), 3, device=out.device)
        i = 0
        for im in images:
            k = im.shape[0]
            if bn:
                ops.stem_conv(im.contiguous(), ps, bias=shift, scale=scale, relu=True, out=out[i:i + k])
            else:
                ops.stem_conv(im.contiguous(), ps, bias=self.conv1.bias.detach(), relu=False, stats=stats[i:i + k], out=out[i:i + k])
            i += k
        if bn:
            return out, None
        if self.layer1[0].takes_raw_input(out):
            return out, ops.instnorm_finalize(stats, (hh // 2) * (ww // 2), eps=self.norm1.eps, channels=64)
        return ops.instnorm_apply(out, stats, eps=self.norm1.eps, relu=True), None

    def _final(self, x, split_act, valid=None):
        m = self.conv2
        b, _, hh, ww = x.shape
        half = m.out_channels // 2
        if ww % 4 == 0 and x.is_contiguous():
            def pack():
                w, bv = m.weight.detach(), m.bias.detach()
                return ops.Conv1x1(w, bv), ops.Conv1x1(w[:half].contiguous(), bv[:half].contiguous()), ops.Conv1x1(w[half:].contiguous(), bv[half:].contiguous())
            whole, lo, hi = _cached(self, '_final_packed', wkey(m.weight, m.bias), pack)
            out = torch.empty(b, m.out_channels, hh, ww, device=x.device)
            if not split_act:
                whole(x, ops.CONV_LINEAR, out, x3=CONV_BF16X3, valid=valid)
            else:
                lo(x, ops.CONV_TANH, out[:, :half], valid=valid)
                hi(x, ops.CONV_RELU, out[:, half:], x3=CONV_BF16X3, valid=valid)
            if valid is not None:
                self._ws['out'] = out
                return ops.copy_rect(out, torch.empty(b, m.out_channels, *valid, device=x.device), *valid)
            return out
        y = ops.conv_direct(x, m.weight, m.bias, 1, 0)
        if split_act:
            y[:, :half] = torch.tanh(y[:, :half])
            ops.bias_act(y[:, half:].contiguous(), None, relu=True, out=y, out_offset=half)
        return y

    def _apply(self, fn, *a, **k):
        r = super()._apply(fn, *a, **k)
        self.__dict__.pop('_key_tensors', None)
        if getattr(self, '_recorded', None) is not None:
            self._recorded.clear()
        return r

    def forward(self, x, raw255=False, split_act=False, route=None):
        images = list(x) if isinstance(x, (list, tuple)) else [x]
        first = images[0]
        if route is None:
            route = resolve_route(pad_encoders=self.pad_encoders, image_size=first.shape[-2:])
        if FRAME_OPLISTS and raw255 and first.is_cuda and first.device.index == torch.cuda.current_device() and not torch.is_grad_enabled() \
                and sum(im.shape[0] for im in images) <= FRAME_OPLISTS_MAX_IMAGES \
                and all(im.is_contiguous() and im.dtype == torch.float32 and im.device == first.device for im in images) and not _overlap(images):
            recorded, wkey = _recording(self, self)
            key = (tuple(tuple(im.shape) for im in images), first.device.index, ops.raw_stream(), split_act, _switches(), self.training, wkey, route.options)
            rec = recorded.get(key)
            if rec is not None:
                out = torch.empty(rec.out_shape, device=first.device)
                rec.replay({**{i: im for i, im in enumerate(images)}, 'out': out})
                return out
            if recorded.wanted(key):
                rec = ops.Recorder()
                with rec:
                    out = self._forward(x, raw255, split_act, route.enc_pad)
                if rec.complete and out.is_contiguous():
                    for i, im in enumerate(images):
                        rec.complete = rec.complete and rec.bind(i, im) > 0
                    rec.complete = rec.complete and rec.bind('out', out) > 0
                    rec.out_shape = tuple(out.shape)
                recorded.put(key, rec)
                return out
        return self._forward(x, raw255, split_act, route.enc_pad)

    def _forward(self, x, raw255, split_act, padded):
        many = isinstance(x, (list, tuple))
        first = x[0] if many else x
        hh, ww = first.shape[-2:]
        stem_ok = raw255 and hh % 2 == 0 and ww % 2 == 0 and ((hh // 2) * (ww // 2)) % 4 == 0 and isinstance(self.norm1, (nn.BatchNorm2d, nn.InstanceNorm2d))
        x_norm = None
        if stem_ok:
            x, x_norm = self._stem_many(list(x) if many else [x])
        else:
            x = (torch.cat(list(x), dim=0) if many else x).contiguous()
            x = conv_norm_act(self.conv1, self.norm1, 2 * (x / 255.0) - 1.0 if raw255 else x, relu=True)
        x = self.layer1[1](self.layer1[0](x, x_norm))
        if padded is None:
            x = self.layer3(self.layer2(x))
            return self._final(x, split_act)
        (hp, wp), h8, w8 = padded, hh // 8, ww // 8
        ws = self._ws = dict(valid=(h8, w8), p2=self._p2(x.shape[0], 4 * hp, 4 * wp, (4 * h8, 4 * w8), x.device))
        x = ops.copy_rect(x, ws['p2'], 4 * h8, 4 * w8)
        for name, layer, v in (('l2', self.layer2, (2 * h8, 2 * w8)), ('l3', self.layer3, (h8, w8))):
            ws[name] = x = layer[1](layer[0](x, valid=v), valid=v)
        return self._final(x, split_act, valid=(h8, w8))

    def _padded(self, hh, ww):
        return resolve_route(pad_encoders=self.pad_encoders, image_size=(hh, ww)).enc_pad

    def _p2(self, n, h2, w2, content, device):
        cache = self.__dict__.setdefault('_p2_cache', {})
        key = (n, h2, w2, content, str(device))
        if key not in cache:
            bounded_put(cache, key, torch.zeros(n, 64, h2, w2, device=device), keep=2)
        return cache[key]


class FlowHead(nn.Module):
    def __init__(self, input_dim=128, hidden_dim=256):
        super().__init__()
        self.conv1 = nn.Conv2d(input_dim, hidden_dim, 3, padding=1)
        self.conv2 = nn.Conv2d(hidden_dim, 2, 3, padding=1)
        self.relu = nn.ReLU(inplace=True)

    def forward(self, x):
        return self.conv2(self.relu(self.conv1(x)))


class SepConvGRU(nn.Module):

    def __init__(self, hidden_dim=128, input_dim=192 + 128):
        super().__init__()
        c = hidden_dim + input_dim
        self.convz1 = nn.Conv2d(c, hidden_dim, (1, 5), padding=(0, 2))
        self.convr1 = nn.Conv2d(c, hidden_dim, (1, 5), padding=(0, 2))
        self.convq1 = nn.Conv2d(c, hidden_dim, (1, 5), padding=(0, 2))
        self.convz2 = nn.Conv2d(c, hidden_dim, (5, 1), padding=(2, 0))
        self.convr2 = nn.Conv2d(c, hidden_dim, (5, 1), padding=(2, 0))
        self.convq2 = nn.Conv2d(c, hidden_dim, (5, 1), padding=(2, 0))


class BasicMotionEncoder(nn.Module):
    def __init__(self, corr_levels=4, corr_radius=4):
        super().__init__()
        cor_planes = corr_levels * (2 * corr_radius + 1) ** 2
        self.convc1 = nn.Conv2d(cor_planes, 256, 1, padding=0)
        self.convc2 = nn.Conv2d(256, 192, 3, padding=1)
        self.convf1 = nn.Conv2d(2, 128, 7, padding=3)
        self.convf2 = nn.Conv2d(128, 64, 3, padding=1)
        self.conv = nn.Conv2d(64 + 192, 128 - 2, 3, padding=1)

    def flow_branch(self, flow, P, L):
        ops.stem_conv(flow, P['convf1'], bias=self.convf1.bias.detach(), relu=True, div=1.0, mul=1.0, sub=0.0, out=L.flo, **L.vk)
        L.f2()

    def forward(self, flow, corr, cat_buf, hx, rhx):
        def cv(m, x):
            return ops.conv_direct(x, m.weight, None, m.stride, m.padding)
        cor = ops.bias_act(cv(self.convc1, corr), self.convc1.bias)
        ops.bias_act(cv(self.convc2, cor), self.convc2.bias, out=cat_buf, out_offset=0)
        flo = ops.bias_act(cv(self.convf1, flow), self.convf1.bias)
        ops.bias_act(cv(self.convf2, flo), self.convf2.bias, out=cat_buf, out_offset=192)
        ops.bias_act(cv(self.conv, cat_buf), self.conv.bias, out=hx, out_offset=128, out2=rhx, out2_offset=128)
        ops.bias_act(flow, None, relu=False, out=hx, out_offset=254, out2=rhx, out2_offset=254)


class BasicUpdateBlock(nn.Module):
    def __init__(self, corr_levels=4, corr_radius=4, hidden_dim=128):
        super().__init__()
        self.hidden_dim = hidden_dim
        self.route = resolve_route()
        self.encoder = BasicMotionEncoder(corr_levels, corr_radius)
        self.gru = SepConvGRU(hidden_dim=hidden_dim, input_dim=128 + hidden_dim)
        self.flow_head = FlowHead(hidden_dim, hidden_dim=256)
        self.mask = nn.Sequential(nn.Conv2d(128, 256, 3, padding=1), nn.ReLU(inplace=True),
                                  nn.Conv2d(256, 64 * 9, 1, padding=0))

    def gate_weights(self, with_key=False):
        g, c = self.gru, self.hidden_dim

        def split(w):
            return torch.cat((w[:, :c], w[:, 2 * c:]), 1).detach().contiguous(), w[:, c:2 * c].detach().contiguous()
# ... 216 lines not shown
                              map_size, image_size)
        ub = self.update_block
        if ub.route[:6] != route[:6]:
            ub.route = route.options
        return route

    def _padded(self, h8, w8):
        return self._route(map_size=(h8, w8)).loop_pad

    def _check_update_fp16(self, w8):
        self._route(map_size=(w8, w8))

    def _pyramid(self, route, b, h8, w8, device):
        p = self._pyr
        if route.alternate_corr:
            c = self.fnet.conv2.out_channels
            if not isinstance(p, ops.AltCorr) or (p.b, p.c, p.h8, p.w8, p.fp16) != (b, c, h8, w8, route.alt_corr_fp16) or p.buf.device != device:
                self._pyr = p = ops.AltCorr(b, c, h8, w8, self.corr_levels, self.corr_radius, device=device, fp16=route.alt_corr_fp16)
            return p
        x3 = CORR_BF16X3 or CONV_BF16X3
        if p is None or (p.b, p.h8, p.w8) != (b, h8, w8) or p.buf.device != device or getattr(p, 'x3', False) != x3:
            self._pyr = ops.CorrPyramid(b, h8, w8, self.corr_levels, self.corr_radius, device=device, bf16x3=x3)
            self._pyr.x3 = x3
        return self._pyr

    def _workspace(self, n, h8, w8, device, padded=None):
        key = (n, h8, w8, str(device), padded)
        if self._ws is None:
            self._ws = {}
        if key not in self._ws:
            if len(self._ws) >= 2:
                self._ws.pop(next(iter(self._ws)))
            c = self.hidden_dim
            mh, mw = (h8, w8) if padded is None else padded
            e = lambda ch: (torch.empty if padded is None else torch.zeros)(n, ch, mh, mw, device=device)
            self._ws[key] = dict(hx=e(2 * c), rhx=e(2 * c), z=e(c), cat=e(2 * c),
                                 corr=e(self.corr_levels * (2 * self.corr_radius + 1) ** 2),
                                 ctx=dict(zr1=e(2 * c), q1=e(c), zr2=e(2 * c), q2=e(c)),
                                 coords0=coords_grid(n, mh, mw, device), coords1=e(2), flow=e(2),
                                 zero2=torch.zeros(n, 2, mh, mw, device=device), valid=None if padded is None else (h8, w8))
            if padded is not None:
                self._ws[key].update(inp=e(c), finit=e(2))
        return self._ws[key]

    def _loop_program(self, pyr, ws, iters, side):
        launchers_key, L = self.update_block.launchers(ws, pyr, with_key=True)
        key = (launchers_key, iters, None if side is None else side[0].cuda_stream)
        return _cached(ws, '_program', key, lambda: self._make_loop_program(L, iters, side))

    def _make_loop_program(self, L, iters, side):
        lk, c1 = (L.lookup, L.c1) if L.lookup_c1 is None else (L.lookup_c1, None)
        prog = ops.OpList(n_cells=2 + 2 * iters)
        if side is not None:
            for cell, ev in ((0, side[1]), (1, side[2])):
                ev.record()
                prog.cells[cell] = ev.cuda_event
        marks = []
        for itr in range(iters):
            marks.append(prog.mark())
            if side is not None:
                prog.record(0, 0).wait(0, 1).add(L.f1, 1).add(L.f2, 1).record(1, 1)
            prog.record(2 + 2 * itr, 0).add(lk).record(3 + 2 * itr, 0)
            if c1 is not None:
                prog.add(c1)
            prog.add(L.c2)
            if side is not None:
                prog.wait(1, 0)
            else:
                prog.add(L.f1).add(L.f2)
            prog.add(L.cv)
            for launch in L.gru:
                prog.add(launch)
        marks.append(prog.mark())
        prog.keep = side
        prog.armed = False
        return prog, marks

    def _encode(self, net, images, route=None, **kw):
        if route is None:
            first = images[0] if isinstance(images, (list, tuple)) else images
            route = self._route(image_size=None if first is None else first.shape[-2:])
        return net(images, raw255=True, route=route, **kw)

    @torch.no_grad()
    def encode_features(self, images):
        return self._encode(self.fnet, images).float()

    @torch.no_grad()
    def encode_context(self, images):
        return self._encode(self.cnet, images, split_act=True)

    @torch.no_grad()
    def encode_both(self, feature_images, context_images):
        many = isinstance(context_images, (list, tuple))
        first = context_images[0] if many else context_images
        count = sum(t.shape[0] for t in context_images) if many else first.shape[0]
        if not (ENC_STREAMS and first.is_cuda and count >= ENC_STREAMS_MIN):
            return self.encode_features(feature_images), self.encode_context(context_images)
        stream, ev_in, ev_done = self._side_stream(first.device)
        cur = torch.cuda.current_stream(first.device)
        ev_in.record(cur)
        with torch.cuda.stream(stream):
            stream.wait_event(ev_in)
            cn = self.encode_context(context_images)
            ev_done.record(stream)
        f = self.encode_features(feature_images)
        cur.wait_event(ev_done)
        cn.record_stream(cur)
        return f, cn

    def _begin(self, route, pyr, ws, fmap1, fmap2, cnet, fused, flow_init=None):
        c = self.hidden_dim
        if route.alternate_corr:
            pyr.build(fmap1.float(), fmap2.float())
        else:
            pyr.build(fmap1.float(), fmap2.float(), fp16_features=route.mixed_precision, bf16x3=(CORR_BF16X3 or CONV_BF16X3) and not route.mixed_precision)
        hx, rhx = ws['hx'], ws['rhx']
        if ws['valid'] is not None:
            h8, w8 = ws['valid']
            ops.copy_rect(cnet[:, :c], hx[:, :c], h8, w8)
            ops.copy_rect(cnet[:, c:], ws['inp'], h8, w8)
            ctx = self.update_block.context_terms(ws['inp'], out=ws['ctx'])
            if flow_init is not None:
                flow_init = ops.copy_rect(flow_init, ws['finit'], h8, w8)
        else:
            ops.copy_planes(cnet[:, :c], hx[:, :c])
            ctx = self.update_block.context_terms(cnet[:, c:], out=ws['ctx'] if fused else None)
        if fused and flow_init is not None:
            ops.flow_seed(flow_init, coords_out=ws['coords1'], flow_out=ws['flow'], dst1=hx[:, 2 * c - 2:], dst2=rhx[:, 2 * c - 2:])
        elif fused:
            ops.copy_planes(ws['coords0'], ws['coords1'])
            ops.copy_planes(ws['zero2'], ws['flow'])
            ops.copy_planes(ws['zero2'], hx[:, 2 * c - 2:])
            ops.copy_planes(ws['zero2'], rhx[:, 2 * c - 2:])
        return ctx

    def _prediction(self, flow, hx, upsample, valid=None):
        if upsample:
            return ops.upsample_convex(flow, self.update_block.up_mask(hx[:, :self.hidden_dim]), size=valid)
        if valid is not None:
            return ops.copy_rect(flow, torch.empty(flow.shape[0], 2, *valid, device=flow.device), *valid)
        return ops.copy_planes(flow, torch.empty_like(flow))

    def _finish(self, ws, upsample, ret_lowres=False):
        c = self.hidden_dim
        hx, flow, valid = ws['hx'], ws['flow'], ws['valid']
        pred = self._prediction(flow, hx, upsample, valid)
        if valid is not None:
            fresh = lambda ch: torch.empty(hx.shape[0], ch, *valid, device=hx.device)
            return pred, ops.copy_rect(hx[:, :c], fresh(c), *valid), ops.copy_rect(flow, fresh(2), *valid) if ret_lowres else None
        h_buf = ops.copy_planes(hx[:, :c], torch.empty(hx.shape[0], c, hx.shape[2], hx.shape[3], device=hx.device))
        low = ops.copy_planes(flow, torch.empty_like(flow)) if ret_lowres else None
        return pred, h_buf, low

    def _run_loop(self, pyr, ws, iters, side):
        prog, marks = self._loop_program(pyr, ws, iters, side)
        if LOOKUP_EVENT_SINK is not None:
            for i, h in enumerate(LOOKUP_EVENT_SINK(iters)):
                prog.cells[2 + i] = h
            prog.armed = True
        elif prog.armed:
            for i in range(2 * iters):
                prog.cells[2 + i] = None
            prog.armed = False
        streams = (ops.raw_stream(),) if side is None else (ops.raw_stream(), side[0].cuda_stream)
        return prog, marks, streams

    def _forward_recorded(self, route, fmap1, fmap2, cnet, iters, upsample, flow_init=None, ret_lowres=False):
        N, _, h8, w8 = fmap1.shape
        dev = fmap1.device
        c = self.hidden_dim
        ts = (fmap1, fmap2, cnet) + (() if flow_init is None else (flow_init,))
        if not all(ops._is_f32(t) and t.device == dev for t in ts) or _overlap(ts) \
                or tuple(cnet.shape) != (N, 2 * c, h8, w8) or dev.index != torch.cuda.current_device() \
                or (flow_init is not None and tuple(flow_init.shape) != (N, 2, h8, w8)):
            return None
        recorded, wkey = _recording(self, self.update_block)
        pyr = self._pyramid(route, N, h8, w8, dev)
        ws = self._workspace(N, h8, w8, dev, route.loop_pad)
        key = (N, h8, w8, dev.index, ops.raw_stream(), iters, upsample, flow_init is not None, ret_lowres, route.options, _switches(),
               pyr.buf.data_ptr(), ws['hx'].data_ptr(), wkey)
        ins = {'f1': fmap1, 'f2': fmap2, 'cnet': cnet}
        if flow_init is not None:
            ins['finit'] = flow_init
        side = self._side_stream(dev) if SIDE_STREAM and N * h8 * w8 <= SIDE_STREAM_MAX else None
        entry = recorded.get(key)
        if entry is not None:
            pre, post = entry.pre, entry
            pre.replay(ins)
# ... 181 lines not shown
```

Baseline: 248.9 pose solves/s.

## Write fmap2 patch layout directly from encoder final conv into corr pyramid

The feature encoder's final 1x1 conv now also stores the fmap2 rows straight into the correlation pyramid's permuted patch-tiled buffer, zero-filling any padding tiles. The later corr build detects this and skips the separate k_permute_fmap pass over fmap2. This removes one full read and write of fmap2 per frame pair. In exchange the epilogue does extra scattered stores, and the shortcut depends on weakref and pointer bookkeeping to confirm the pyramid still holds data from the same tensor.

```diff
diff --git a/include/rpe.h b/include/rpe.h
--- a/include/rpe.h
+++ b/include/rpe.h
@@ -154,6 +154,7 @@
                    void *pyramid, void *stream);
 int rpe_corr_build_ex(const float *fmap1, const float *fmap2, int b, int c, int h8, int w8, int levels, int feature_dtype,
                       void *pyramid, void *stream);
+int rpe_corr_build_pre(const float *fmap1, int b, int c, int h8, int w8, int levels, void *pyramid, void *stream);
 int rpe_corr_lookup(const void *pyramid, const float *coords, int b, int h8, int w8, int levels, int radius,
                     float *out, void *stream);
 int rpe_corr_lookup_ex(const void *pyramid, const float *coords, int b, int h8, int w8, int levels, int radius, int map_h, int map_w,
@@ -265,6 +266,8 @@
 size_t rpe_conv1x1_packed_floats(int cout, int cin);
 int rpe_conv1x1_pack(const float *weight, int cout, int cin, float *packed, void *stream);
 int rpe_conv1x1(const rpe_conv_desc *desc, void *stream);
+typedef struct rpe_conv_desc_p { rpe_conv_desc d; void *pyramid; int pairs, levels, row_lo, row_hi; } rpe_conv_desc_p;
+int rpe_conv1x1_patch(const rpe_conv_desc_p *desc, void *stream);
 size_t rpe_conv1x1_x3_packed_bytes(int cout, int cin);
 int rpe_conv1x1_x3_pack(const float *weight, int cout, int cin, void *packed, void *stream);
 int rpe_conv1x1_x3(const rpe_conv_desc *desc, void *stream);
@@ -325,6 +328,8 @@
 #define RPE_OP_CORR_ALT_PREPARE_EX 39
 #define RPE_OP_CORR_ALT_LOOKUP_DT 40
 #define RPE_OP_CONV_F16 (RPE_OP_CORR_ALT_LOOKUP_DT + 1)
+#define RPE_OP_CONV1X1_PATCH (RPE_OP_CONV_F16 + 1)
+#define RPE_OP_CORR_BUILD_PRE (RPE_OP_CONV_F16 + 2)
 typedef struct rpe_op {
     int kind;
     int stream;
@@ -336,6 +341,7 @@
     long long out_batch_stride; float *out2; long long out2_batch_stride;
 } rpe_lookup_conv1x1_args;
 typedef struct rpe_corr_build_args { const float *fmap1, *fmap2; int b, c, h8, w8, levels, feature_dtype; void *pyramid; } rpe_corr_build_args;
+typedef struct rpe_corr_build_pre_args { const float *fmap1; int b, c, h8, w8, levels; void *pyramid; } rpe_corr_build_pre_args;
 typedef struct rpe_corr_alt_prepare_args { const float *fmap1, *fmap2; int b, c, h8, w8, levels; void *scratch; } rpe_corr_alt_prepare_args;
 typedef struct rpe_corr_alt_lookup_args { const void *scratch; const float *coords; int b, c, h8, w8, levels, radius; float *out; } rpe_corr_alt_lookup_args;
 typedef struct rpe_stem_conv_args {
diff --git a/robust-pose-estimator_amd/_lib.py b/robust-pose-estimator_amd/_lib.py
--- a/robust-pose-estimator_amd/_lib.py
+++ b/robust-pose-estimator_amd/_lib.py
@@ -27,6 +27,10 @@
     _fields_ = [('h_valid', _i), ('w_valid', _i)]
 
 
+class ConvDescP(ConvDesc):
+    _fields_ = [('pyramid', _vp), ('pairs', _i), ('levels', _i), ('row_lo', _i), ('row_hi', _i)]
+
+
 def struct_fields(st):
     return [f for cls in reversed(type(st).__mro__) for f in cls.__dict__.get('_fields_', ())]
 
@@ -49,6 +53,10 @@
 
 class CorrBuildArgs(_c.Structure):
     _fields_ = [('fmap1', _vp), ('fmap2', _vp), ('b', _i), ('c', _i), ('h8', _i), ('w8', _i), ('levels', _i), ('feature_dtype', _i), ('pyramid', _vp)]
+
+
+class CorrBuildPreArgs(_c.Structure):
+    _fields_ = [('fmap1', _vp), ('b', _i), ('c', _i), ('h8', _i), ('w8', _i), ('levels', _i), ('pyramid', _vp)]
 
 
 class CorrAltPrepareArgs(_c.Structure):
@@ -141,6 +149,7 @@
 OP_ENC_CONV_WINO_V, OP_ENC_CONV_WINO24_V, OP_ENC_CONV_S2_V, OP_ENC_CONV_S2_M96_V, OP_INSTNORM_APPLY_V = 34, 35, 36, 37, 38
 OP_CORR_ALT_PREPARE_EX, OP_CORR_ALT_LOOKUP_DT = 39, 40
 OP_CONV_F16 = 41
+OP_CONV1X1_PATCH, OP_CORR_BUILD_PRE = 42, 43
 F32, F16 = 0, 2
 LIST_OPS = {OP_CONV_FUSED: ('rpe_conv_fused', ConvDesc), OP_CONV_WINO: ('rpe_conv_wino', ConvDesc), OP_CONV_WINO1D: ('rpe_conv_wino1d', ConvDesc),
             OP_CONV1X1: ('rpe_conv1x1', ConvDesc), OP_CONV_WINO_X3: ('rpe_conv_wino_x3', ConvDesc),
@@ -164,7 +173,8 @@
             'rpe_conv_fused_m96': 'rpe_enc_conv_s2_m96_v'}
 LIST_OPS_ALT_DT = {OP_CORR_ALT_PREPARE_EX: ('rpe_corr_alt_prepare_ex', CorrAltPrepareExArgs), OP_CORR_ALT_LOOKUP_DT: ('rpe_corr_alt_lookup_dt', CorrAltLookupDtArgs)}
 LIST_OPS_F16 = {OP_CONV_F16: ('rpe_conv_f16', ConvDesc)}
-ALL_LIST_OPS = {**LIST_OPS, **LIST_OPS_ENC, **LIST_OPS_ALT_DT, **LIST_OPS_F16}
+LIST_OPS_PATCH = {OP_CONV1X1_PATCH: ('rpe_conv1x1_patch', ConvDesc), OP_CORR_BUILD_PRE: ('rpe_corr_build_pre', CorrBuildPreArgs)}
+ALL_LIST_OPS = {**LIST_OPS, **LIST_OPS_ENC, **LIST_OPS_ALT_DT, **LIST_OPS_F16, **LIST_OPS_PATCH}
 KIND_OF_ENTRY = {entry: kind for kind, (entry, _) in ALL_LIST_OPS.items()}
 
 ABI_MINOR = 3
diff --git a/robust-pose-estimator_amd/csrc/conv1x1.hip b/robust-pose-estimator_amd/csrc/conv1x1.hip
--- a/robust-pose-estimator_amd/csrc/conv1x1.hip
+++ b/robust-pose-estimator_amd/csrc/conv1x1.hip
@@ -16,6 +16,7 @@
     float* out; long long obs; float* out2; long long o2bs;
     int mode;
     int W, Hv, Wv;
+    float* pp; int p_lo, p_hi, p_npx, p_np;
 };
 
 __device__ __forceinline__ void dma16_2v(const float* base, unsigned v0, unsigned v1, unsigned lds_addr) {
@@ -35,7 +36,7 @@
 
 __host__ __device__ __forceinline__ int g1_chan(int rho) { return (rho >> 1) + 8 * (rho & 1); }
 
-template <int MODE, bool OUT2, bool VALID = false>
+template <int MODE, bool OUT2, bool VALID = false, bool PATCH = false>
 __global__ __launch_bounds__(256, G1_OCC) void k_conv1x1(G1P P) {
     __shared__ __attribute__((aligned(16))) float As[3][G1_TILE];
     __shared__ __attribute__((aligned(16))) float Bs[3][G1_TILE];
@@ -141,6 +142,8 @@
     float* ob2 = OUT2 ? P.out2 + (size_t)bz * P.o2bs : nullptr;
     const int co_w = co0 + wm * 64;
     const int cout = P.cout;
+    const bool dual = PATCH && bz >= P.p_lo && bz < P.p_hi;
+    float* pb = dual ? P.pp + (size_t)(bz - P.p_lo) * cout * P.p_np : nullptr;
     const float* bsl = &bias_s[wm * 64 + 4 * lh];
 #pragma unroll
     for (int j = 0; j < 2; ++j) {
@@ -148,6 +151,11 @@
         const bool pok = px < hw;
         const bool pvalid = !VALID || (px / P.W < P.Hv && px % P.W < P.Wv);
         const unsigned loff = ((unsigned)(4 * lh) * (unsigned)hw + (unsigned)px) * 4u;
+        unsigned poff = 0;
+        if (PATCH) {
+            const int y = px / P.W, x = px - y * P.W;
+            poff = ((unsigned)(4 * lh) * (unsigned)P.p_np + (unsigned)(((y >> 3) * P.p_npx + (x >> 4)) * 128 + (y & 7) * 16 + (x & 15))) * 4u;
+        }
 #pragma unroll
         for (int i = 0; i < 2; ++i)
 #pragma unroll
@@ -164,8 +172,18 @@
 #endif
                     store_sv(ob + (size_t)row_u * hw, loff, v);
                     if (OUT2) store_sv(ob2 + (size_t)row_u * hw, loff, v);
+                    if (PATCH && dual) store_sv(pb + (size_t)row_u * P.p_np, poff, v);
                 }
             }
+    }
+    if (PATCH && dual && P.p_np != hw) {
+        const int H = hw / P.W, ntile = gridDim.x / ncot;
+        for (int n = (int)(lid / ncot) * 128 + (tid & 127); n < P.p_np; n += ntile * 128) {
+            const int t = n >> 7, r = n & 127;
+            const int y = (t / P.p_npx) * 8 + (r >> 4), x = (t % P.p_npx) * 16 + (r & 15);
+            if (y >= H || x >= P.W)
+                for (int co = co0 + (tid >> 7); co < co0 + G1_M && co < cout; co += 2) pb[(size_t)co * P.p_np + n] = 0.0f;
+        }
     }
 }
 
@@ -188,7 +206,9 @@
     return launch_pack(k_conv1x1_pack, weight, packed, cout, cin, 1, (long long)rpe_conv1x1_packed_floats(cout, cin), stream, ceil_div(cin, G1_K));
 }
 
-static int conv1x1_launch(const rpe_conv_desc* d, int hv, int wv, void* stream) {
+bool rpe_corr_patch_dst(int b, int c, int h8, int w8, int levels, void* pyramid, float** bp, int* npx, int* np);
+
+static int conv1x1_launch(const rpe_conv_desc* d, int hv, int wv, void* stream, const rpe_conv_desc_p* dp = nullptr) {
     if (!conv_desc_present(d)) return RPE_E_BADARG;
     if (d->kh != 1 || d->kw != 1 || !stride_is_1(d)) return RPE_E_UNSUPPORTED;
     if (!conv_linear_or_relu(d) && d->mode != RPE_CONV_TANH) return RPE_E_UNSUPPORTED;
@@ -199,8 +219,18 @@
     G1P P;
     fill_common(P, d, round_up(d->cout, 128));
     P.hw = (int)hw; P.W = d->w; P.Hv = hv; P.Wv = wv;
+    P.pp = nullptr; P.p_lo = P.p_hi = P.p_npx = P.p_np = 0;
     const bool valid = hv != d->h || wv != d->w;
     const dim3 grid(ceil_div(hw, G1_N) * (P.coP / 128), 1, d->b);
+    if (dp) {
+        if (d->mode != RPE_CONV_LINEAR || d->out2 || valid) return RPE_E_UNSUPPORTED;
+        if (dp->row_lo < 0 || dp->row_hi > d->b || dp->row_hi - dp->row_lo != dp->pairs) return RPE_E_BADARG;
+        if (!rpe_corr_patch_dst(dp->pairs, d->cout, d->h, d->w, dp->levels, dp->pyramid, &P.pp, &P.p_npx, &P.p_np)) return RPE_E_BADARG;
+        if ((long long)P.p_np * 16 * 4 >= (1ll << 32)) return RPE_E_UNSUPPORTED;
+        P.p_lo = dp->row_lo; P.p_hi = dp->row_hi;
+        hipLaunchKernelGGL((k_conv1x1<RPE_CONV_LINEAR, false, false, true>), grid, dim3(256), 0, (hipStream_t)stream, P);
+        return rpe_check_launch();
+    }
 #define G1_LAUNCH(M_) do { if (valid && d->out2) hipLaunchKernelGGL((k_conv1x1<M_, true, true>), grid, dim3(256), 0, (hipStream_t)stream, P); \
                            else if (valid) hipLaunchKernelGGL((k_conv1x1<M_, false, true>), grid, dim3(256), 0, (hipStream_t)stream, P); \
                            else if (d->out2) hipLaunchKernelGGL((k_conv1x1<M_, true>), grid, dim3(256), 0, (hipStream_t)stream, P); \
@@ -218,3 +248,8 @@
     if (!dv || !conv_valid_extent_ok(dv)) return RPE_E_BADARG;
     return conv1x1_launch(&dv->d, dv->h_valid, dv->w_valid, stream);
 }
+
+extern "C" int rpe_conv1x1_patch(const rpe_conv_desc_p* dp, void* stream) {
+    if (!dp || !dp->pyramid) return RPE_E_BADARG;
+    return conv1x1_launch(&dp->d, dp->d.h, dp->d.w, stream, dp);
+}
diff --git a/robust-pose-estimator_amd/csrc/corr.hip b/robust-pose-estimator_amd/csrc/corr.hip
--- a/robust-pose-estimator_amd/csrc/corr.hip
+++ b/robust-pose-estimator_amd/csrc/corr.hip
@@ -1056,6 +1056,8 @@
     }
 }
 
+static int build_f32(const float* fmap1, const float* fmap2, int b, int c, int h8, int w8, const PyrGeom& G, float* pyr, hipStream_t s);
+
 extern "C" int rpe_corr_build_ex(const float* fmap1, const float* fmap2, int b, int c, int h8, int w8, int levels, int feature_dtype,
                                  void* pyramid, void* stream) {
     PyrGeom G;
@@ -1065,7 +1067,6 @@
     hipStream_t s = (hipStream_t)stream;
     float* pyr = (float*)pyramid;
     float* Ap = pyr + G.total;
-    float* Bp = Ap + (size_t)b * c * G.mp;
     if (feature_dtype == RPE_F16) {
         half4* Ah = (half4*)Ap;
         half4* Bh = Ah + (size_t)b * (c / 4) * G.mp;
@@ -1084,9 +1085,15 @@
                            1.0f / sqrtf((float)c), G);
         return rpe_check_launch();
     }
+    return build_f32(fmap1, fmap2, b, c, h8, w8, G, pyr, s);
+}
+
+static int build_f32(const float* fmap1, const float* fmap2, int b, int c, int h8, int w8, const PyrGeom& G, float* pyr, hipStream_t s) {
+    float* Ap = pyr + G.total;
+    float* Bp = Ap + (size_t)b * c * G.mp;
     const bool a_in_place = (w8 % 8 == 0) && G.mp == h8 * w8 && (((uintptr_t)fmap1) & 15) == 0;
     if (!a_in_place) hipLaunchKernelGGL(k_permute_fmap, dim3(ceil_div(G.mp, 256), b * c), dim3(256), 0, s, fmap1, Ap, h8, w8, 0, G.gx, G.npx, G.mp);
-    hipLaunchKernelGGL(k_permute_fmap, dim3(ceil_div(G.np, 256), b * c), dim3(256), 0, s, fmap2, Bp, h8, w8, 1, G.gx, G.npx, G.np);
+    if (fmap2) hipLaunchKernelGGL(k_permute_fmap, dim3(ceil_div(G.np, 256), b * c), dim3(256), 0, s, fmap2, Bp, h8, w8, 1, G.gx, G.npx, G.np);
 #ifndef CB_SMALL_WG
 #define CB_SMALL_WG 4096
 #endif
@@ -1098,6 +1105,21 @@
     hipLaunchKernelGGL(k_corr_build<true>, dim3(G.nbands, G.mp / BM, b), dim3(256), 0, s, a_in_place ? fmap1 : (const float*)Ap, (const float*)Bp, pyr, c,
                        1.0f / sqrtf((float)c), G);
     return rpe_check_launch();
+}
+
+bool rpe_corr_patch_dst(int b, int c, int h8, int w8, int levels, void* pyramid, float** bp, int* npx, int* np) {
+    PyrGeom G;
+    if (!pyramid || (((uintptr_t)pyramid) & 15) || c <= 0 || c > 256 || c % BK != 0 || !make_geom(b, h8, w8, levels, G)) return false;
+    *bp = (float*)pyramid + G.total + (size_t)b * c * G.mp;
+    *npx = G.npx; *np = G.np;
+    return true;
+}
+
+extern "C" int rpe_corr_build_pre(const float* fmap1, int b, int c, int h8, int w8, int levels, void* pyramid, void* stream) {
+    PyrGeom G;
+    if (!fmap1 || !pyramid || c <= 0 || c > 256 || c % BK != 0 || !make_geom(b, h8, w8, levels, G)) return RPE_E_BADARG;
+    if (((uintptr_t)pyramid) & 15) return RPE_E_BADARG;
+    return build_f32(fmap1, nullptr, b, c, h8, w8, G, (float*)pyramid, (hipStream_t)stream);
 }
 
 extern "C" int rpe_corr_build(const float* fmap1, const float* fmap2, int b, int c, int h8, int w8, int levels,
diff --git a/robust-pose-estimator_amd/csrc/oplist.hip b/robust-pose-estimator_amd/csrc/oplist.hip
--- a/robust-pose-estimator_amd/csrc/oplist.hip
+++ b/robust-pose-estimator_amd/csrc/oplist.hip
@@ -24,6 +24,8 @@
 static_assert(sizeof(rpe_instnorm_apply_v_args) == 72, "rpe_instnorm_apply_v_args: layout changed -- update _lib.py and RPE_ABI_VERSION");
 static_assert(sizeof(rpe_corr_alt_prepare_ex_args) == 48, "rpe_corr_alt_prepare_ex_args: layout changed -- update _lib.py and RPE_ABI_VERSION");
 static_assert(sizeof(rpe_corr_alt_lookup_dt_args) == 64, "rpe_corr_alt_lookup_dt_args: layout changed -- update _lib.py and RPE_ABI_VERSION");
+static_assert(sizeof(rpe_conv_desc_p) == 224, "rpe_conv_desc_p: layout changed -- update _lib.py and RPE_ABI_VERSION");
+static_assert(sizeof(rpe_corr_build_pre_args) == 40, "rpe_corr_build_pre_args: layout changed -- update _lib.py and RPE_ABI_VERSION");
 static_assert(sizeof(rpe_solve_opts) == 32, "rpe_solve_opts: layout changed -- update _lib.py and RPE_ABI_VERSION");
 
 template <typename A>
@@ -143,6 +145,11 @@
         return rpe_corr_alt_lookup_dt(a->scratch, a->coords, a->b, a->c, a->h8, a->w8, a->levels, a->radius, a->map_h, a->map_w, a->feature_dtype,
                                       a->out, st);
     }
+    case RPE_OP_CONV1X1_PATCH: return rpe_conv1x1_patch(as<rpe_conv_desc_p>(op), st);
+    case RPE_OP_CORR_BUILD_PRE: {
+        const auto* a = as<rpe_corr_build_pre_args>(op);
+        return rpe_corr_build_pre(a->fmap1, a->b, a->c, a->h8, a->w8, a->levels, a->pyramid, st);
+    }
     case RPE_OP_EVENT_RECORD: {
         hipEvent_t ev = (hipEvent_t) * static_cast<void* const*>(op.args);
         if (!ev) return RPE_OK;
diff --git a/robust-pose-estimator_amd/ops.py b/robust-pose-estimator_amd/ops.py
--- a/robust-pose-estimator_amd/ops.py
+++ b/robust-pose-estimator_amd/ops.py
@@ -1,5 +1,6 @@
 import ctypes
 import operator
+import weakref
 
 import torch
 
@@ -487,6 +488,16 @@
         if nbytes == 0:
             raise _lib.RpeError('rpe_corr_pyramid_bytes: unsupported geometry')
         self.buf = torch.empty(nbytes, dtype=torch.uint8, device=device)
+        self.patch_src = None
+
+    def _holds(self, f2):
+        note, self.patch_src = self.patch_src, None
+        src = None if note is None or _REC is not None else note[0]()
+        if src is None:
+            return False
+        lo, hi = note[1], note[2]
+        return f2.is_contiguous() and tuple(f2.shape) == (hi - lo,) + tuple(src.shape[1:]) \
+            and f2.data_ptr() == src.data_ptr() + lo * src.stride(0) * src.element_size()
 
     def build(self, fmap1, fmap2, fp16_features=False, bf16x3=False):
         f1, f2 = _dev(fmap1, torch.float32, 'fmap1'), _dev(fmap2, torch.float32, 'fmap2')
@@ -496,6 +507,8 @@
         mode = 2 if fp16_features else 3 if bf16x3 else 0
         if self.buf.numel() < lib().rpe_corr_pyramid_bytes_ex(b, h8, w8, self.levels, mode):
             raise _lib.RpeError('corr build: this pyramid was not sized for the requested feature mode (CorrPyramid(..., bf16x3=True))')
+        if self._holds(f2) and mode == 0:
+            return _launch(_lib.OP_CORR_BUILD_PRE, (ptr(f1), b, c, h8, w8, self.levels, ptr(self.buf)), (f1, f2, self), self)
         return _launch(_lib.OP_CORR_BUILD, (ptr(f1), ptr(f2), b, c, h8, w8, self.levels, mode, ptr(self.buf)), (f1, f2, self), self)
 
     def lookup(self, coords, out=None, prepare=False, map_size=None):
@@ -865,6 +878,24 @@
     return conv_fused(x, pc, mode, out, out2=out2, prepare=prepare, entry=pc.entry, valid=valid)
 
 
+def conv1x1_patch(x, pc, out, pyr, rows):
+    lo, hi = rows
+    b, _, hh, ww = x.shape
+    if not isinstance(pyr, CorrPyramid) or (pyr.b, pyr.h8, pyr.w8) != (hi - lo, hh, ww) or not 0 <= lo < hi <= b:
+        raise _lib.RpeError(f'conv1x1_patch: rows {rows} of a batch of {b} {hh}x{ww} maps do not fill this pyramid')
+    if not out.is_contiguous() or tuple(out.shape) != (b, pc.cout, hh, ww):
+        raise _lib.RpeError('conv1x1_patch: out must be the contiguous (b, cout, h, w) map the build reads fmap1 from')
+    d0, bias, _ = _conv_desc('conv1x1_patch', x, pc, CONV_LINEAR, dict(out=out), _PLAIN_RULES, None, 'packed', None, None, modes=(CONV_LINEAR,),
+                             tile_major=False, kernel=(pc.kh, pc.kw))
+    d = _lib.ConvDescP()
+    ctypes.memmove(ctypes.byref(d), ctypes.byref(d0), ctypes.sizeof(d0))
+    d.pyramid, d.pairs, d.levels, d.row_lo, d.row_hi = pyr.buf.data_ptr(), hi - lo, pyr.levels, lo, hi
+    pyr.patch_src = None
+    r = _launch(_lib.OP_CONV1X1_PATCH, d, (x, pc, out, bias, pyr), out)
+    pyr.patch_src = (weakref.ref(out), lo, hi)
+    return r
+
+
 class Conv1x1:
 
     def __init__(self, weight, bias=None):
@@ -884,7 +915,7 @@
     gemm_x3 = property(lambda self: self._packing(PackedConv1x1X3))
     f16 = property(lambda self: self._packing(PackedConvF16))
 
-    def __call__(self, x, mode, out, out2=None, prepare=False, x3=False, valid=None, f16=False):
+    def __call__(self, x, mode, out, out2=None, prepare=False, x3=False, valid=None, f16=False, patch=None):
         b, _, hh, ww = x.shape
         if f16:
             if x3 or valid is not None:
@@ -898,6 +929,10 @@
             if not aligned or x3:
                 raise _lib.RpeError('Conv1x1: a valid extent needs the f32 GEMM route (16-byte aligned input slice, h * w % 4 == 0, no bf16x3)')
             return conv1x1(x, self.gemm, mode, out, out2=out2, prepare=prepare, valid=valid)
+        if big and patch is not None and mode == CONV_LINEAR and out2 is None and not prepare and not x3 and out.is_contiguous() \
+                and self.cout % 16 == 0 and self.cout <= 256 and isinstance(patch[0], CorrPyramid) \
+                and (patch[0].b, patch[0].h8, patch[0].w8) == (patch[2] - patch[1], hh, ww):
+            return conv1x1_patch(x, self.gemm, out, patch[0], patch[1:])
         if big:
             return conv1x1(x, self.gemm, mode, out, out2=out2, prepare=prepare)
         return conv_fused(x, self.fused, mode, out, out2=out2, prepare=prepare)
diff --git a/robust-pose-estimator_amd/pose_net.py b/robust-pose-estimator_amd/pose_net.py
--- a/robust-pose-estimator_amd/pose_net.py
+++ b/robust-pose-estimator_amd/pose_net.py
@@ -126,9 +126,11 @@
         return self
 
     @torch.no_grad()
-    def _encode_both(self, feature_images, context_images):
+    def _encode_both(self, feature_images, context_images, fmap2_rows=None):
         both = getattr(self.flow, 'encode_both', None)
         if both is not None:
+            if fmap2_rows is not None and hasattr(self.flow, '_fmap2_patch'):
+                return both(feature_images, context_images, fmap2_rows=fmap2_rows)
             return both(feature_images, context_images)
         return self.flow.encode_features(feature_images), self.flow.encode_context(context_images)
 
@@ -158,7 +160,7 @@
         intrinsics = intrinsics.expand(n, 3, 3).contiguous()
         baseline = baseline.expand(n).contiguous()
         if cache1 is None:
-            f, cn = self._encode_both((image1l, image2l, image2r), (image1l, image2l))
+            f, cn = self._encode_both((image1l, image2l, image2r), (image1l, image2l), fmap2_rows=(n, 3 * n))
             f2l = f[n:2 * n]
             fmaps = (f[:2 * n], f[n:])
             c2l = cn[n:]
diff --git a/robust-pose-estimator_amd/raft.py b/robust-pose-estimator_amd/raft.py
--- a/robust-pose-estimator_amd/raft.py
+++ b/robust-pose-estimator_amd/raft.py
@@ -29,6 +29,7 @@
 FRAME_OPLISTS_MAX_IMAGES = 4
 ENC_STREAMS = True
 ENC_STREAMS_MIN = 8
+FMAP2_FROM_ENCODER = True
 SIDE_STREAM_MAX = 8 * 5120
 ROUTE_SWITCHES = ('WINOGRAD', 'WINO_2X4', 'S2_M96', 'S2_M96_MIN_WGS', 'CORR_BF16X3', 'CONV_BF16X3', 'X3_MIN_CIN', 'X3_GRU', 'SIDE_STREAM', 'SIDE_STREAM_MAX',
                   'LOOKUP_FUSED', 'LOOKUP_FUSED_MAX_WGS', 'ENC_STREAMS', 'ENC_STREAMS_MIN', 'PAD_MAPS', 'PAD_ENCODERS', 'UPDATE_FP16')
@@ -316,7 +317,7 @@
             return out, ops.instnorm_finalize(stats, (hh // 2) * (ww // 2), eps=self.norm1.eps, channels=64)
         return ops.instnorm_apply(out, stats, eps=self.norm1.eps, relu=True), None
 
-    def _final(self, x, split_act, valid=None):
+    def _final(self, x, split_act, valid=None, patch=None):
         m = self.conv2
         b, _, hh, ww = x.shape
         half = m.out_channels // 2
@@ -327,7 +328,7 @@
             whole, lo, hi = _cached(self, '_final_packed', wkey(m.weight, m.bias), pack)
             out = torch.empty(b, m.out_channels, hh, ww, device=x.device)
             if not split_act:
-                whole(x, ops.CONV_LINEAR, out, x3=CONV_BF16X3, valid=valid)
+                whole(x, ops.CONV_LINEAR, out, x3=CONV_BF16X3, valid=valid, patch=patch)
             else:
                 lo(x, ops.CONV_TANH, out[:, :half], valid=valid)
                 hi(x, ops.CONV_RELU, out[:, half:], x3=CONV_BF16X3, valid=valid)
@@ -348,7 +349,7 @@
             self._recorded.clear()
         return r
 
-    def forward(self, x, raw255=False, split_act=False, route=None):
+    def forward(self, x, raw255=False, split_act=False, route=None, patch=None):
         images = list(x) if isinstance(x, (list, tuple)) else [x]
         first = images[0]
         if route is None:
@@ -374,9 +375,9 @@
                     rec.out_shape = tuple(out.shape)
                 recorded.put(key, rec)
                 return out
-        return self._forward(x, raw255, split_act, route.enc_pad)
-
-    def _forward(self, x, raw255, split_act, padded):
+        return self._forward(x, raw255, split_act, route.enc_pad, patch)
+
+    def _forward(self, x, raw255, split_act, padded, patch=None):
         many = isinstance(x, (list, tuple))
         first = x[0] if many else x
         hh, ww = first.shape[-2:]
@@ -390,7 +391,7 @@
         x = self.layer1[1](self.layer1[0](x, x_norm))
         if padded is None:
             x = self.layer3(self.layer2(x))
-            return self._final(x, split_act)
+            return self._final(x, split_act, patch=patch)
         (hp, wp), h8, w8 = padded, hh // 8, ww // 8
         ws = self._ws = dict(valid=(h8, w8), p2=self._p2(x.shape[0], 4 * hp, 4 * wp, (4 * h8, 4 * w8), x.device))
         x = ops.copy_rect(x, ws['p2'], 4 * h8, 4 * w8)
@@ -773,21 +774,33 @@
             route = self._route(image_size=None if first is None else first.shape[-2:])
         return net(images, raw255=True, route=route, **kw)
 
+    def _fmap2_patch(self, images, rows):
+        if rows is None or not FMAP2_FROM_ENCODER or CORR_BF16X3 or CONV_BF16X3:
+            return None
+        first = images[0] if isinstance(images, (list, tuple)) else images
+        route = self._route(image_size=first.shape[-2:])
+        if route.alternate_corr or route.mixed_precision or route.enc_pad is not None or not first.is_cuda:
+            return None
+        if first.shape[-2] % 8 or first.shape[-1] % 8:
+            return None
+        lo, hi = rows
+        return self._pyramid(route, hi - lo, first.shape[-2] // 8, first.shape[-1] // 8, first.device), lo, hi
+
     @torch.no_grad()
-    def encode_features(self, images):
-        return self._encode(self.fnet, images).float()
+    def encode_features(self, images, fmap2_rows=None):
+        return self._encode(self.fnet, images, patch=self._fmap2_patch(images, fmap2_rows)).float()
 
     @torch.no_grad()
     def encode_context(self, images):
         return self._encode(self.cnet, images, split_act=True)
 
     @torch.no_grad()
-    def encode_both(self, feature_images, context_images):
+    def encode_both(self, feature_images, context_images, fmap2_rows=None):
         many = isinstance(context_images, (list, tuple))
         first = context_images[0] if many else context_images
         count = sum(t.shape[0] for t in context_images) if many else first.shape[0]
         if not (ENC_STREAMS and first.is_cuda and count >= ENC_STREAMS_MIN):
-            return self.encode_features(feature_images), self.encode_context(context_images)
+            return self.encode_features(feature_images, fmap2_rows), self.encode_context(context_images)
         stream, ev_in, ev_done = self._side_stream(first.device)
         cur = torch.cuda.current_stream(first.device)
         ev_in.record(cur)
@@ -795,7 +808,7 @@
             stream.wait_event(ev_in)
             cn = self.encode_context(context_images)
             ev_done.record(stream)
-        f = self.encode_features(feature_images)
+        f = self.encode_features(feature_images, fmap2_rows)
         cur.wait_event(ev_done)
         cn.record_stream(cur)
         return f, cn
```

Result: no change. 249.2 pose solves/s, median of 4 (+0.1%).
